# rubenwiersma/gravo_mg

Hardware: AMD Instinct MI355X
Metric: V-cycle wall time (ms per V-cycle incl. residual check) + solve-to-1e-4 iterations, 3M-vertex Poisson (lower is better)
Workload: dtype f64

## Files before the change

### gravo_mg_amd/cabi.py

```python
from __future__ import annotations

import ctypes as C
import os
from typing import List, Optional, Sequence, Tuple

import numpy as np
import scipy.sparse as sp

_HERE = os.path.dirname(os.path.abspath(__file__))
LIB_PATH = os.environ.get("GMG_LIB_PATH") or os.path.join(_HERE, "lib", "libgravomg_hip.so")

GMG_OK, GMG_ERR_INVALID, GMG_ERR_NO_DEVICE, GMG_ERR_HIP, GMG_ERR_STATE, GMG_ERR_NUMERIC, GMG_ERR_UNSUPPORTED = 0, -1, -2, -3, -4, -5, -6
DIVERGED = 1
SMOOTHER_MULTICOLOR_GS, SMOOTHER_JACOBI, SMOOTHER_CHEBYSHEV = 0, 1, 2
COARSE_HOST_LDLT, COARSE_DEVICE_INVERSE, COARSE_AUTO, COARSE_DEVICE_TRIANGLE = 0, 1, 2, 3

_STATUS_NAMES = {
    -1: "GMG_ERR_INVALID", -2: "GMG_ERR_NO_DEVICE", -3: "GMG_ERR_HIP", -4: "GMG_ERR_STATE",
    -5: "GMG_ERR_NUMERIC", -6: "GMG_ERR_UNSUPPORTED",
}


class GmgError(RuntimeError):
    def __init__(self, code: int, msg: str):
        super().__init__(f"{_STATUS_NAMES.get(code, code)}: {msg}")
        self.code = code


class GmgConfig(C.Structure):
    _fields_ = [
        ("device", C.c_int), ("smoother", C.c_int), ("jacobi_omega", C.c_double), ("pre_iters", C.c_int),
        ("post_iters", C.c_int), ("coarse_mode", C.c_int), ("use_graph", C.c_int), ("sigma", C.c_int),
        ("row_align", C.c_int), ("block_rows", C.c_int), ("block_lanes", C.c_int), ("block_from_level", C.c_int),
        ("device_setup", C.c_int), ("device_rap", C.c_int), ("reorder_fine", C.c_int), ("inner_precision", C.c_int), ("block_csr", C.c_int), ("host_threads", C.c_int),
        ("verbose", C.c_int), ("gs_omega", C.c_double), ("restrict_sigma", C.c_int), ("block_ep", C.c_int), ("dist_shard_levels", C.c_int), ("block_fine", C.c_int), ("fine_col16", C.c_int), ("stream_gate", C.c_int), ("dist_exchange", C.c_int), ("prepare_structure", C.c_int), ("fuse_restrict_sweep", C.c_int), ("speculate_head", C.c_int), ("uniform_slices", C.c_int), ("color_ahead", C.c_int),
        ("accelerate", C.c_int),
    ]


class GmgHierarchyOptions(C.Structure):
    _fields_ = [
        ("ratio", C.c_double), ("lower_bound", C.c_int), ("check_voronoi", C.c_int), ("nested", C.c_int),
        ("sampling", C.c_int), ("weighting", C.c_int), ("debug", C.c_int), ("full_clustering", C.c_int), ("use_device", C.c_int),
    ]


class GmgDeviceVectors(C.Structure):
    _fields_ = [
        ("rhs", C.c_void_p), ("rhs_row_stride", C.c_int64), ("rhs_col_stride", C.c_int64),
        ("x0", C.c_void_p), ("x0_row_stride", C.c_int64), ("x0_col_stride", C.c_int64),
        ("x", C.c_void_p), ("x_row_stride", C.c_int64), ("x_col_stride", C.c_int64),
    ]


_ip = C.POINTER(C.c_int)
_dp = C.POINTER(C.c_double)
_vp = C.c_void_p

SIGNATURES = {
    "gmg_config_default": (C.c_int, [C.POINTER(GmgConfig)]),
    "gmg_config_size": (C.c_int, []),
    "gmg_create": (C.c_int, [C.POINTER(GmgConfig), C.POINTER(_vp)]),
    "gmg_destroy": (None, [_vp]),
    "gmg_last_error": (C.c_char_p, [_vp]),
    "gmg_device_count": (C.c_int, []),
    "gmg_set_num_levels": (C.c_int, [_vp, C.c_int]),
    "gmg_set_prolongation": (C.c_int, [_vp, C.c_int, C.c_int, C.c_int, _ip, _ip, _dp]),
    "gmg_set_mass": (C.c_int, [_vp, C.c_int, _dp]),
    "gmg_set_system": (C.c_int, [_vp, C.c_int, _ip, _ip, _dp]),
    "gmg_num_levels": (C.c_int, [_vp]),
    "gmg_level_info": (C.c_int, [_vp, C.c_int, _ip, C.POINTER(C.c_int64), _ip, _ip]),
    "gmg_get_level_operator": (C.c_int, [_vp, C.c_int, _ip, _ip, _dp]),
    "gmg_get_level_ordering": (C.c_int, [_vp, C.c_int, _ip, _ip]),
    "gmg_get_level_blocks": (C.c_int, [_vp, C.c_int, _ip, _ip, C.POINTER(C.c_ubyte)]),
    "gmg_get_timing": (C.c_int, [_vp, C.c_char_p, _dp]),
    "gmg_smooth": (C.c_int, [_vp, C.c_int, _dp, _dp, C.c_int, C.c_int]),
    "gmg_residual": (C.c_int, [_vp, C.c_int, _dp, _dp, C.c_int, _dp]),
    "gmg_spmv": (C.c_int, [_vp, C.c_int, _dp, C.c_int, _dp]),
    "gmg_restrict": (C.c_int, [_vp, C.c_int, _dp, C.c_int, _dp]),
    "gmg_prolong_add": (C.c_int, [_vp, C.c_int, _dp, C.c_int, _dp]),
    "gmg_coarse_solve": (C.c_int, [_vp, _dp, C.c_int, _dp]),
    "gmg_residual_norm": (C.c_int, [_vp, _dp, _dp, C.c_int, C.c_int, _dp]),
    "gmg_vcycle": (C.c_int, [_vp, _dp, _dp, C.c_int]),
    "gmg_smooth_residual": (C.c_int, [_vp, C.c_int, _dp, _dp, C.c_int, C.c_int, C.c_int, _dp]),
    "gmg_solve": (C.c_int, [_vp, _dp, _dp, C.c_int, C.c_double, C.c_int, C.c_int, _ip, _dp, _dp]),
    "gmg_solve_x0_rhs": (C.c_int, [_vp, _dp, _dp, C.c_int, C.c_double, C.c_int, C.c_int, _ip, _dp, _dp]),
    "gmg_solve_device": (C.c_int, [_vp, C.POINTER(GmgDeviceVectors), C.c_int, C.c_double, C.c_int, C.c_int, _ip, _dp, _dp]),
    "gmg_set_system_values_device": (C.c_int, [_vp, C.c_void_p, C.c_int64]),
    "gmg_load_problem": (C.c_int, [_vp, _dp, _dp, C.c_int]),
    "gmg_run_cycles": (C.c_int, [_vp, C.c_int, C.c_int, _dp]),
    "gmg_fetch_solution": (C.c_int, [_vp, _dp]),
    "gmg_set_stream": (C.c_int, [_vp, _vp]),
    "gmg_dist_setup": (C.c_int, [_vp, C.c_int, C.c_int]),
    "gmg_dist_partition": (C.c_int, [_vp, C.c_int, C.c_int]),
    "gmg_dist_bind": (C.c_int, [_vp, _vp, _vp, _vp, C.c_int]),
    "gmg_dist_smooth_color": (C.c_int, [_vp, C.c_int]),
    "gmg_dist_residual_own": (C.c_int, [_vp]),
    "gmg_dist_coarse_cycle": (C.c_int, [_vp]),
    "gmg_dist_prolong_own": (C.c_int, [_vp]),
    "gmg_dist_norm_partial": (C.c_int, [_vp, C.c_int, _dp]),
    "gmg_dist_all_rows": (C.c_int, [_vp, C.c_int]),
    "gmg_dist_gather": (C.c_int, [_vp, C.c_void_p, C.c_void_p, C.c_int64, C.c_void_p]),
    "gmg_dist_scatter": (C.c_int, [_vp, C.c_void_p, C.c_void_p, C.c_void_p, C.c_int64, C.c_void_p]),
    "gmg_p2p_blob_bytes": (C.c_int, []),
    "gmg_p2p_prepare": (C.c_int, [_vp, C.c_int, C.c_int, C.c_int]),
    "gmg_p2p_export": (C.c_int, [_vp, C.c_void_p]),
    "gmg_p2p_connect": (C.c_int, [_vp, C.c_void_p]),
    "gmg_p2p_rccl_unique_id": (C.c_int, [C.c_void_p]),
    "gmg_p2p_connect_rccl": (C.c_int, [_vp, C.c_void_p]),
    "gmg_p2p_load": (C.c_int, [_vp, _dp, _dp]),
    "gmg_p2p_cycles": (C.c_int, [_vp, C.c_int, C.c_int, _dp]),
    "gmg_p2p_fetch": (C.c_int, [_vp, _dp]),
    "gmg_p2p_solve": (C.c_int, [_vp, _dp, _dp, C.c_double, C.c_int, C.c_int, C.POINTER(C.c_int), C.POINTER(C.c_double)]),
    "gmg_p2p_stat": (C.c_int, [_vp, C.c_char_p, _dp]),
    "gmg_p2p_set_smoother": (C.c_int, [_vp, C.c_int]),
    "gmg_p2p_set_fences": (C.c_int, [_vp, C.c_int]),
    "gmg_hierarchy_options_default": (C.c_int, [C.POINTER(GmgHierarchyOptions)]),
    "gmg_hierarchy_build": (C.c_int, [_dp, C.c_int, _ip, C.c_int, C.POINTER(GmgHierarchyOptions), C.POINTER(_vp)]),
    "gmg_hierarchy_destroy": (None, [_vp]),
# ... 118 lines not shown


def _pd(a: np.ndarray):
    return a.ctypes.data_as(_dp)


class Hierarchy:

    def __init__(self, pos, neigh, ratio=8.0, lower_bound=1000, check_voronoi=True, nested=False, sampling=0, weighting=0, debug=False, full_clustering=False, use_device=True):
        l = lib()
        pos = np.ascontiguousarray(pos, dtype=np.float64)
        neigh = np.ascontiguousarray(neigh, dtype=np.int32)
        if pos.ndim != 2 or pos.shape[1] != 3 or neigh.ndim != 2 or neigh.shape[0] != pos.shape[0]:
            raise ValueError("pos must be n x 3 and neigh n x K")
        opt = GmgHierarchyOptions()
        l.gmg_hierarchy_options_default(C.byref(opt))
        opt.ratio, opt.lower_bound, opt.check_voronoi, opt.nested = float(ratio), int(lower_bound), int(bool(check_voronoi)), int(bool(nested))
        opt.sampling, opt.weighting, opt.debug, opt.full_clustering = int(sampling), int(weighting), int(bool(debug)), int(bool(full_clustering))
        opt.use_device = int(use_device)
        self._h = _vp()
        rc = l.gmg_hierarchy_build(_pd(pos), pos.shape[0], _pi(neigh), neigh.shape[1], C.byref(opt), C.byref(self._h))
        if rc:
            raise GmgError(rc, "gmg_hierarchy_build failed (only Sampling.FASTDISK is supported)" if rc == GMG_ERR_UNSUPPORTED else "gmg_hierarchy_build failed")
        self.U: List[sp.csc_matrix] = []
        for k in range(l.gmg_hierarchy_num_levels(self._h)):
            nf, nc, nnz = C.c_int(), C.c_int(), C.c_int()
            l.gmg_hierarchy_level_shape(self._h, k, C.byref(nf), C.byref(nc), C.byref(nnz))
            colptr = np.empty(nc.value + 1, np.int32); rowidx = np.empty(nnz.value, np.int32); val = np.empty(nnz.value, np.float64)
            l.gmg_hierarchy_get_prolongation(self._h, k, _pi(colptr), _pi(rowidx), _pd(val))
            self.U.append(sp.csc_matrix((val, rowidx, colptr), shape=(nf.value, nc.value)))
        self.samples, self.nearest, self.points = [], [], []
        for k, u in enumerate(self.U):
            s_ = np.empty(u.shape[1], np.int32); n_ = np.empty(u.shape[0], np.int32); p_ = np.empty((u.shape[1], 3), np.float64)
            if l.gmg_hierarchy_get_samples(self._h, k, _pi(s_)) or l.gmg_hierarchy_get_nearest(self._h, k, _pi(n_)) or l.gmg_hierarchy_get_points(self._h, k, _pd(p_)):
                raise GmgError(GMG_ERR_INVALID, "hierarchy getters failed")
            self.samples.append(s_); self.nearest.append(n_); self.points.append(p_)
        self.triangles = []
        for k in range(len(self.U)):
            cnt = C.c_int()
            l.gmg_hierarchy_get_triangles(self._h, k, None, C.byref(cnt))
            t = np.empty((cnt.value, 3), np.int32)
            if cnt.value:
                l.gmg_hierarchy_get_triangles(self._h, k, _pi(t), C.byref(cnt))
            self.triangles.append(t)
        cnt = C.c_int()
        l.gmg_hierarchy_get_fine_order(self._h, None, C.byref(cnt))
        self.fine_order = None
        if cnt.value:
            self.fine_order = np.empty(cnt.value, np.int32)
            l.gmg_hierarchy_get_fine_order(self._h, _pi(self.fine_order), C.byref(cnt))

    def row_kinds(self, k: int) -> np.ndarray:
        out = np.zeros(4, np.int32)
        if lib().gmg_hierarchy_debug_row_kinds(self._h, int(k), _pi(out)):
            raise GmgError(GMG_ERR_INVALID, "gmg_hierarchy_debug_row_kinds failed")
        return out

    def timing(self, key: str) -> float:
        out = C.c_double()
        rc = lib().gmg_hierarchy_get_timing(self._h, key.encode(), C.byref(out))
        if rc:
            raise KeyError(key)
        return out.value

    TIMING_KEYS = ("n_vertices", "hierarchy", "sampling", "cluster", "next_neighborhood", "next_positions",
                   "triangle_finding", "triangle_selection", "PDS", "levels")

    def timings(self) -> dict:
        return {k: self.timing(k) for k in self.TIMING_KEYS}

    def __del__(self):
        try:
            if getattr(self, "_h", None):
                lib().gmg_hierarchy_destroy(self._h)
                self._h = None
        except Exception:
            pass


class Engine:

    def __init__(self, smoother=SMOOTHER_MULTICOLOR_GS, pre_iters=2, post_iters=2, jacobi_omega=0.67,
                 coarse_mode=COARSE_AUTO, use_graph=False, sigma=0, row_align=64, block_rows=64, block_from_level=1, block_lanes=0,
                 device_setup=True, device_rap=True, reorder_fine=2, inner_precision=0, block_csr=True, device=0, verbose=False, gs_omega=None, block_ep=None, restrict_sigma=None, dist_shard_levels=None, block_fine=None, fine_col16=None, stream_gate=None, prepare_structure=None, dist_exchange=None, fuse_restrict_sweep=None, speculate_head=None, uniform_slices=None, color_ahead=None, accelerate=0):
        l = lib()
        cfg = GmgConfig()
        l.gmg_config_default(C.byref(cfg))
        cfg.device, cfg.smoother, cfg.jacobi_omega = int(device), int(smoother), float(jacobi_omega)
        cfg.pre_iters, cfg.post_iters, cfg.coarse_mode = int(pre_iters), int(post_iters), int(coarse_mode)
        cfg.use_graph, cfg.sigma, cfg.row_align, cfg.verbose = int(bool(use_graph)), int(sigma), int(row_align), int(bool(verbose))
        cfg.block_rows, cfg.block_from_level, cfg.block_lanes = int(block_rows), int(block_from_level), int(block_lanes)
        cfg.device_setup, cfg.device_rap, cfg.reorder_fine = int(bool(device_setup)), int(bool(device_rap)), int(reorder_fine)
        cfg.inner_precision, cfg.block_csr = int(inner_precision), int(bool(block_csr))
        if gs_omega is not None:
            cfg.gs_omega = float(gs_omega)
        if block_ep is not None:
            cfg.block_ep = int(bool(block_ep))
        if restrict_sigma is not None:
            cfg.restrict_sigma = int(restrict_sigma)
        if dist_shard_levels is not None:
            cfg.dist_shard_levels = int(dist_shard_levels)
        if block_fine is not None:
            cfg.block_fine = int(bool(block_fine))
        if fine_col16 is not None:
            cfg.fine_col16 = int(bool(fine_col16))
        if stream_gate is not None:
            cfg.stream_gate = int(bool(stream_gate))
        if prepare_structure is not None:
            cfg.prepare_structure = int(bool(prepare_structure))
        if fuse_restrict_sweep is not None:
            cfg.fuse_restrict_sweep = int(bool(fuse_restrict_sweep))
        if speculate_head is not None:
            cfg.speculate_head = int(bool(speculate_head))
        if uniform_slices is not None:
            cfg.uniform_slices = int(bool(uniform_slices))
        if color_ahead is not None:
            cfg.color_ahead = int(bool(color_ahead))
        if dist_exchange is not None:
            cfg.dist_exchange = int(dist_exchange)
        cfg.accelerate = int(accelerate)
        self._h = _vp()
        rc = l.gmg_create(C.byref(cfg), C.byref(self._h))
        if rc:
            raise GmgError(rc, "gmg_create failed (invalid configuration)")
        self._n0 = None
        self._sizes: List[int] = []
        self.pre_iters, self.post_iters = int(pre_iters), int(post_iters)
        self.gs_omega = float(cfg.gs_omega)

    @classmethod
    def borrow(cls, handle: int) -> "Engine":
        self = cls.__new__(cls)
        self._h = _vp(int(handle))
        self._borrowed = True
        self._n0 = None
        self._sizes = []
        self.pre_iters = self.post_iters = None
        self.gs_omega = None
        return self

    def _chk(self, rc: int):
        if rc:
            raise GmgError(rc, lib().gmg_last_error(self._h).decode())

    def close(self):
        if getattr(self, "_h", None):
            if not getattr(self, "_borrowed", False):
                lib().gmg_destroy(self._h)
            self._h = None

    def __del__(self):
        try:
            self.close()
        except Exception:
            pass

    def set_prolongations(self, U: Sequence, finalize: bool = True, fine_order=None, fine_graph=None):
        l = lib()
        self._chk(l.gmg_set_num_levels(self._h, len(U)))
        self._sizes = []
        for k, u in enumerate(U):
            u = _csc(u)
            self._chk(l.gmg_set_prolongation(self._h, k, u.shape[0], u.shape[1], _pi(u.indptr), _pi(u.indices), _pd(u.data)))
            if k == 0:
                self._sizes.append(u.shape[0])
            self._sizes.append(u.shape[1])
        if fine_order is not None and len(U):
            fo = np.ascontiguousarray(fine_order, dtype=np.int32)
            self._chk(l.gmg_set_fine_order(self._h, fo.shape[0], _pi(fo)))
        if fine_graph is not None and len(U):
            fg = np.ascontiguousarray(fine_graph, dtype=np.int32)
            self._chk(l.gmg_set_fine_graph(self._h, fg.shape[0], fg.shape[1], _pi(fg)))
        if finalize and len(U):
            self._chk(l.gmg_finalize_hierarchy(self._h))

    def use_hierarchy(self, hier: Hierarchy):
        self._chk(lib().gmg_use_hierarchy(self._h, hier._h))
        self._sizes = [hier.U[0].shape[0]] + [u.shape[1] for u in hier.U] if hier.U else []

    def set_mass(self, mass_diag):
        m = np.ascontiguousarray(mass_diag, dtype=np.float64).ravel()
        self._chk(lib().gmg_set_mass(self._h, m.shape[0], _pd(m)))

    def set_system(self, lhs):
        a = _csc_layout(lhs)
        if a.shape[0] != a.shape[1]:
            raise ValueError("lhs must be square")
        self._chk(lib().gmg_set_system(self._h, a.shape[0], _pi(a.indptr), _pi(a.indices), _pd(a.data)))
        self._n0 = a.shape[0]

    @property
    def num_levels(self) -> int:
        return int(lib().gmg_num_levels(self._h))

    def level_info(self, k: int) -> dict:
        n, nnz, nc, npad = C.c_int(), C.c_int64(), C.c_int(), C.c_int()
        self._chk(lib().gmg_level_info(self._h, k, C.byref(n), C.byref(nnz), C.byref(nc), C.byref(npad)))
        return {"n": n.value, "nnz": nnz.value, "n_colors": nc.value, "n_pad": npad.value}

    def level_operator(self, k: int) -> sp.csc_matrix:
        info = self.level_info(k)
        colptr = np.empty(info["n"] + 1, np.int32); rowidx = np.empty(info["nnz"], np.int32); val = np.empty(info["nnz"], np.float64)
        self._chk(lib().gmg_get_level_operator(self._h, k, _pi(colptr), _pi(rowidx), _pd(val)))
# ... 429 lines not shown
```

### gravo_mg_amd/csrc/bindings.cpp

```cpp
#include <chrono>
#include <cstdio>
#include <cstdlib>
#include <pybind11/numpy.h>
#include <pybind11/pybind11.h>
#include <pybind11/stl.h>

#include <algorithm>
#include <atomic>
#include <cmath>
#include <cstdint>
#include <memory>
#include <stdexcept>
#include <string>
#include <thread>
#include <vector>

#include "multigrid_solver.h"

namespace py = pybind11;
using DenseIn = py::array_t<double, py::array::f_style | py::array::forcecast>;
using IntIn = py::array_t<int, py::array::c_style | py::array::forcecast>;

namespace {

// ... 202 lines not shown
        MGBS::MatrixXd x = b;
        solver->clearError();
        if (pardiso) throw std::runtime_error("direct_solve(pardiso=True): Pardiso (MKL) is not part of this build; use pardiso=False (sparse LDL^T)");
        solver->solve(A, b, x, 0);
        check();
        return from_dense(x);
    }

    py::list prolongation_matrices() {
        py::list out;
        for (const auto& u : solver->U) out.append(from_sparse(u));
        return out;
    }

    void set_prolongation_matrices(py::list U) {
        std::vector<MGBS::SparseMatrix> v;
        for (auto item : U) v.push_back(to_sparse(py::reinterpret_borrow<py::object>(item)));
        solver->U = v;
    }

    std::vector<std::vector<int>> sampling_indices() { return solver->samples; }
    std::vector<std::vector<size_t>> nearest_source() { return solver->nearestSource; }
    py::list level_points() {
        py::list out;
        for (const auto& P : solver->levelV) out.append(from_dense(P));
        return out;
    }
    py::list level_edges() { return py::list(); }
    std::vector<std::vector<int>> notrimap() { return solver->noTriFoundMap; }
    std::vector<std::vector<std::vector<int>>> all_triangles() { return solver->allTriangles; }
    py::list coarse_normals() { return py::list(); }

    void write_hierarchy_timing(std::string experiment, std::string file, bool write_headers) { MGBS::writeTiming(solver->hierarchyTiming, experiment, file, write_headers); }
    void write_solver_timing(std::string experiment, std::string file, bool write_headers) { MGBS::writeTiming(solver->solverTiming, experiment, file, write_headers); }
    void write_convergence(std::string file) { MGBS::writeConvergence(solver->convergence, file); }

    double residual(py::object lhs, DenseIn rhs, DenseIn solution, int type = 2) {
        MappedSparse mapped = map_system_matrix(lhs, symCache);
        MGBS::SparseMatrix& A = mapped.m;
        solver->clearError();
        double r = solver->residualCheck(A, to_dense(rhs), to_dense(solution), type);
        check();
        return r;
    }

    std::map<std::string, double> solver_timing() { return solver->solverTiming; }
    std::map<std::string, double> hierarchy_timing() { return solver->hierarchyTiming; }
    std::vector<std::tuple<double, double>> convergence() { return solver->convergence; }
    std::tuple<uintptr_t, long> prepare_system(py::object lhs) {
        MappedSparse mapped = map_system_matrix(lhs, symCache);
        gmg_handle h = nullptr;
        long gen = 0;
        solver->clearError();
        if (solver->prepareSystem(mapped.m, &h, &gen) != GMG_OK) { check(); throw std::runtime_error("prepare_system failed"); }
        return std::make_tuple((uintptr_t)h, gen);
    }
    uintptr_t engine_handle() { return (uintptr_t)solver->engineHandle(); }
    void invalidate_system() { solver->systemChangedExternally(); }
    void set_engine_option(const std::string& key, double value) {
        gmg_config& c = solver->engineConfig;
        if (key == "smoother") c.smoother = (int)value;
        else if (key == "jacobi_omega") c.jacobi_omega = value;
        else if (key == "gs_omega") c.gs_omega = value;
        else if (key == "coarse_mode") c.coarse_mode = (int)value;
        else if (key == "use_graph") c.use_graph = (int)value;
        else if (key == "block_rows") c.block_rows = (int)value;
        else if (key == "block_from_level") c.block_from_level = (int)value;
        else if (key == "device") c.device = (int)value;
        else if (key == "row_align") c.row_align = (int)value;
        else if (key == "block_lanes") c.block_lanes = (int)value;
        else if (key == "dist_shard_levels") c.dist_shard_levels = (int)value;
        else if (key == "block_fine") c.block_fine = (int)value;
        else if (key == "dist_rank") solver->distRank = (int)value;
        else if (key == "dist_world") solver->distWorld = (int)value;
        else if (key == "fine_col16") c.fine_col16 = (int)value;
        else if (key == "stream_gate") c.stream_gate = (int)value;
        else if (key == "fuse_restrict_sweep") c.fuse_restrict_sweep = (int)value;
        else if (key == "speculate_head") c.speculate_head = (int)value;
        else if (key == "uniform_slices") c.uniform_slices = (int)value;
        else if (key == "color_ahead") c.color_ahead = (int)value;
        else if (key == "dist_exchange") c.dist_exchange = (int)value;
        else if (key == "inner_precision") c.inner_precision = (int)value;
        else if (key == "accelerate") c.accelerate = (int)value;
        else throw std::invalid_argument("unknown engine option: " + key);
    }

#ifdef GMG_TESTING
    void test_report_diverged(int n) { solver->testReportDiverged = n; }
#endif

private:
    void check() {
        std::string now = solver->lastError();
        if (!now.empty()) throw std::runtime_error(now);
    }
    std::unique_ptr<MGBS::MultigridSolver> solver;
    SymmetryCache symCache;
};

PYBIND11_MODULE(gravomg_bindings, m) {
    m.doc() = "Multigrid solver bindings (MI355X-native V-cycle hot path)";

    py::enum_<Hierarchy>(m, "Hierarchy").value("OURS", OURS).value("SIG21", SIG21);
    py::enum_<Sampling>(m, "Sampling").value("FASTDISK", FASTDISK).value("POISSONDISK", POISSONDISK).value("FPS", FPS).value("RANDOM", RANDOM).value("MIS", MIS);
    py::enum_<Weighting>(m, "Weighting").value("BARYCENTRIC", BARYCENTRIC).value("UNIFORM", UNIFORM).value("INVDIST", INVDIST);

    py::class_<MultigridSolver>(m, "MultigridSolver")
        .def(py::init<DenseIn, IntIn, py::object, double, int, int, double, int, int, int, int, bool, bool, Sampling, Weighting, bool, DenseIn, bool, bool, bool, int, bool>())
        .def("construct_sig21_hierarchy", &MultigridSolver::construct_sig21_hierarchy, py::arg("F"))
        .def("toggle_hierarchy", &MultigridSolver::toggle_hierarchy, py::arg("hierarchy"))
        .def("solve", &MultigridSolver::solve, py::arg("lhs"), py::arg("rhs"))
        .def("direct_solve", &MultigridSolver::direct_solve, py::arg("lhs"), py::arg("rhs"), py::arg("pardiso"))
        .def("prolongation_matrices", &MultigridSolver::prolongation_matrices)
        .def("set_prolongation_matrices", &MultigridSolver::set_prolongation_matrices, py::arg("U"))
        .def("sampling_indices", &MultigridSolver::sampling_indices)
        .def("level_points", &MultigridSolver::level_points)
        .def("level_edges", &MultigridSolver::level_edges)
        .def("notrimap", &MultigridSolver::notrimap)
        .def("all_triangles", &MultigridSolver::all_triangles)
        .def("coarse_normals", &MultigridSolver::coarse_normals)
        .def("nearest_source", &MultigridSolver::nearest_source)
        .def("write_hierarchy_timing", &MultigridSolver::write_hierarchy_timing, py::arg("experiment"), py::arg("file"), py::arg("write_headers"))
        .def("write_solver_timing", &MultigridSolver::write_solver_timing, py::arg("experiment"), py::arg("file"), py::arg("write_headers"))
        .def("write_convergence", &MultigridSolver::write_convergence, py::arg("file"))
        .def("residual", &MultigridSolver::residual, py::arg("lhs"), py::arg("rhs"), py::arg("solution"), py::arg("type") = 2)
        .def("solver_timing", &MultigridSolver::solver_timing)
        .def("hierarchy_timing", &MultigridSolver::hierarchy_timing)
        .def("convergence", &MultigridSolver::convergence)
        .def("prepare_system", &MultigridSolver::prepare_system, py::arg("lhs"))
        .def("engine_handle", &MultigridSolver::engine_handle)
        .def("invalidate_system", &MultigridSolver::invalidate_system)
        .def("set_engine_option", &MultigridSolver::set_engine_option, py::arg("key"), py::arg("value"))
#ifdef GMG_TESTING
        .def("_test_report_diverged", &MultigridSolver::test_report_diverged, py::arg("n"))
#endif
        ;
}
```

### gravo_mg_amd/csrc/engine.hip

```cpp
#include <hip/hip_runtime.h>
#include <dlfcn.h>

#include <array>
#include <atomic>
#include <chrono>
#include <cmath>
#include <functional>
#include <future>
#include <cstdio>
#include <cstdlib>
#include <cstring>
#include <map>
#include <mutex>
#include <shared_mutex>
#include <string>
#include <vector>

#if !defined(__HIP_DEVICE_COMPILE__)
#include <execinfo.h>
#include <signal.h>
#include <unistd.h>
#endif

#include "../../include/gravomg_hip.h"
// ... 8 lines not shown
#include "setup_kernels.hip.hpp"
#include "hierarchy_kernels.hip.hpp"
#include "accel_kernels.hip.hpp"

using namespace gmg;
using clk = std::chrono::steady_clock;
static inline double ms_since(clk::time_point t0) { return std::chrono::duration<double, std::milli>(clk::now() - t0).count(); }

#if !defined(__HIP_DEVICE_COMPILE__)
namespace {
struct sigaction gmg_prev_action[32];
void gmg_fatal_signal(int sig) {
    void* frames[48];
    const int nf = backtrace(frames, 48);
    const char msg[] = "[gmg] fatal signal, native stack of the faulting thread:\n";
    (void)!write(2, msg, sizeof(msg) - 1);
    backtrace_symbols_fd(frames, nf, 2);
    if (sig > 0 && sig < 32) sigaction(sig, &gmg_prev_action[sig], nullptr); else signal(sig, SIG_DFL);
    raise(sig);
}
struct GmgSignalAid {
    GmgSignalAid() {
        if (!EnvSwitches::get().segv_backtrace) return;
        void* warm[4];
        (void)backtrace(warm, 4);
        struct sigaction sa;
        std::memset(&sa, 0, sizeof(sa));
        sa.sa_handler = gmg_fatal_signal;
        for (int sig : {SIGSEGV, SIGBUS, SIGABRT, SIGFPE}) sigaction(sig, &sa, &gmg_prev_action[sig]);
    }
} gmg_signal_aid;
}
#endif

#include "engine_state.hip.hpp"
#include "engine_setup.hip.hpp"
#include "engine_cycle.hip.hpp"
#include "engine_part.hip.hpp"
#include "engine_system.hip.hpp"

int gate_unwound(gmg_handle h);
#define GMG_CATCH_H                                                                                             \
    catch (const std::exception& e_) { if (h) (void)gate_unwound(h); return h ? fail(h, GMG_ERR_STATE, std::string("exception: ") + e_.what()) : GMG_ERR_STATE; } \
    catch (...) { if (h) (void)gate_unwound(h); return h ? fail(h, GMG_ERR_STATE, "unknown exception") : GMG_ERR_STATE; }
#define GMG_CATCH_0                                              \
    catch (...) { return GMG_ERR_STATE; }

void p2p_release_handle(gmg_handle h);


extern "C" {

int gmg_config_size(void) { return (int)sizeof(gmg_config); }

int gmg_config_default(gmg_config* cfg) try {
    if (!cfg) return GMG_ERR_INVALID;
    std::memset(cfg, 0, sizeof(*cfg));
    cfg->device = 0;
    cfg->smoother = GMG_SMOOTHER_MULTICOLOR_GS;
    cfg->jacobi_omega = 0.67;
    cfg->pre_iters = 2;
    cfg->post_iters = 2;
    cfg->coarse_mode = GMG_COARSE_AUTO;
    cfg->use_graph = 0;
    cfg->sigma = 0;
    cfg->row_align = 64;
    cfg->block_rows = 64;
    cfg->block_from_level = 1;
    cfg->block_lanes = 0;
    cfg->device_setup = 1;
    cfg->device_rap = 1;
    cfg->reorder_fine = 2;
    cfg->inner_precision = 0;
    cfg->block_csr = 1;
    cfg->host_threads = 0;
    cfg->verbose = 0;
    cfg->block_ep = 1;
    cfg->dist_shard_levels = 2;
    cfg->fine_col16 = 1;
    cfg->stream_gate = 1;
    cfg->prepare_structure = 1;
    cfg->fuse_restrict_sweep = 1;
    cfg->speculate_head = 1;
    cfg->uniform_slices = 1;
    cfg->color_ahead = 1;
    cfg->dist_exchange = 0;
    cfg->block_fine = 1;
    cfg->restrict_sigma = 64;
    cfg->gs_omega = 1.35;
    cfg->accelerate = 0;
    return GMG_OK;
} GMG_CATCH_0

int gmg_host_threads(void) try { return hw_threads(); } GMG_CATCH_0

int gmg_device_count(void) try {
    int n = 0;
    if (hipGetDeviceCount(&n) != hipSuccess) return 0;
    return n;
} GMG_CATCH_0

int gmg_create(const gmg_config* cfg, gmg_handle* out) try {
    if (!out) return GMG_ERR_INVALID;
    gmg_config c;
    if (cfg) c = *cfg; else gmg_config_default(&c);
    if (c.sigma < 0 || c.sigma % 64 || c.restrict_sigma < 0 || c.restrict_sigma % 64 || c.row_align <= 0 || c.row_align % 64 || c.pre_iters < 0 || c.post_iters < 0 ||
        c.reorder_fine < 0 || c.reorder_fine > 2 || c.inner_precision < 0 || c.inner_precision > 1 || c.block_rows < 0 || c.block_rows > gmgk::kBlockRows || c.block_rows % 64 || c.block_from_level < 0 || !(c.gs_omega > 0.0 && c.gs_omega < 2.0) || c.dist_shard_levels < 1 || c.dist_shard_levels > 2 || c.block_fine < 0 || c.block_fine > 1 || c.dist_exchange < 0 || c.dist_exchange > 2 ||
        (c.block_lanes != 0 && c.block_lanes != 1 && c.block_lanes != 4) || (c.block_lanes != 1 && c.block_rows > gmgk::kQuadBlockRows)) return GMG_ERR_INVALID;
    if (c.accelerate < 0 || c.accelerate > gmg::kAccelMaxDepth) return GMG_ERR_INVALID;
    if (c.smoother < GMG_SMOOTHER_MULTICOLOR_GS || c.smoother > GMG_SMOOTHER_CHEBYSHEV) return GMG_ERR_INVALID;
    if (c.accelerate > 0 && c.inner_precision) return GMG_ERR_UNSUPPORTED;
    gmg_handle h = new gmg_solver_s();
    h->cfg = c;
    if (h->cfg.host_threads <= 0) h->cfg.host_threads = hw_threads();
    int ndev = gmg_device_count();
    if (ndev > 0 && c.device >= 0 && c.device < ndev && hipSetDevice(c.device) == hipSuccess &&
        hipStreamCreateWithFlags(&h->stream, hipStreamNonBlocking) == hipSuccess) {
        h->has_device = true;
        h->own_stream = h->stream;
        { int cus = 0; if (hipDeviceGetAttribute(&cus, hipDeviceAttributeMultiprocessorCount, c.device) == hipSuccess && cus > 0) h->n_cus = cus; else (void)hipGetLastError(); }
        (void)hipEventCreate(&h->ev0);
        (void)hipEventCreate(&h->ev1);
        if (hipStreamCreateWithFlags(&h->aux_stream, hipStreamNonBlocking) != hipSuccess) { h->aux_stream = nullptr; (void)hipGetLastError(); }
        if (hipEventCreateWithFlags(&h->aux_ev, hipEventDisableTiming) != hipSuccess) { h->aux_ev = nullptr; (void)hipGetLastError(); }
        if (hipMalloc((void**)&h->d_aux_err, sizeof(int)) != hipSuccess) { h->d_aux_err = nullptr; (void)hipGetLastError(); }
        h->poll = EnvSwitches::get().poll;
        (void)ensure_bounce(h);
    }
    *out = h;
    return GMG_OK;
} GMG_CATCH_0

void gmg_destroy(gmg_handle h) {
    if (!h) return;
    PoolScope pool_scope_(&h->pool);
    if (h->has_device) {
        (void)hipSetDevice(h->cfg.device);
        (void)hipStreamSynchronize(h->stream);
        p2p_release_handle(h);
        drop_system(h);
        drop_device_transfers(h);
        h->d_stage = {}; h->d_partials = {}; h->d_norm = {}; h->d_watch = {};
        if (h->h_pinned) (void)sync_hipHostFree(h->h_pinned);
        for (int i = 0; i < 2; ++i) { if (h->h_stage[i]) (void)sync_hipHostFree(h->h_stage[i]); if (h->h_stage_ev[i]) (void)hipEventDestroy(h->h_stage_ev[i]); }
        for (hipEvent_t& e : h->h_chunk_ev) if (e) (void)hipEventDestroy(e);
        if (h->h_norm) (void)sync_hipHostFree(h->h_norm);
        if (h->h_flag) (void)sync_hipHostFree(h->h_flag);
        if (h->ev0) (void)hipEventDestroy(h->ev0);
        if (h->ev1) (void)hipEventDestroy(h->ev1);
        if (h->aux_ev) (void)hipEventDestroy(h->aux_ev);
        if (h->aux_stream) { (void)hipStreamSynchronize(h->aux_stream); (void)sync_hipStreamDestroy(h->aux_stream); }
        if (h->d_aux_err) (void)sync_hipFree(h->d_aux_err);
        drop_rap_order(h);
        for (int i = 0; i < 2; ++i) { if (h->bounce[i]) (void)sync_hipHostFree(h->bounce[i]); if (h->bounce_ev[i]) (void)hipEventDestroy(h->bounce_ev[i]); }
        for (hipEvent_t e : h->prof_ev) (void)hipEventDestroy(e);
        (void)sync_hipStreamDestroy(h->own_stream);
        h->pool.trim();
    }
    delete h;
}

const char* gmg_last_error(gmg_handle h) { return h ? h->err.c_str() : "null handle"; }

int gmg_set_num_levels(gmg_handle h, int L) try {
    if (!h || L < 0 || L > 64) return h ? fail(h, GMG_ERR_INVALID, "invalid level count") : GMG_ERR_INVALID;
    PoolScope pool_scope_(&h->pool);
// ... 300 lines not shown
    if (!e || !x || d <= 0) return fail(h, GMG_ERR_INVALID, "bad arguments");
    if ((rc = ensure_vectors(h, d))) return rc;
    Level& l = h->lv[k];
    if ((rc = to_device(h, k + 1, e, d, h->lv[k + 1].x))) return rc;
    if ((rc = to_device(h, k, x, d, l.x))) return rc;
    launch_prolong_add<double>(h, l, h->lv[k + 1], d, h->lv[k + 1].x, l.x);
    h->loaded_d = 0;
    return to_host(h, k, l.x, d, x);
} GMG_CATCH_H

int gmg_coarse_solve(gmg_handle h, const double* rc_in, int d, double* e) try {
    NEED_DEVICE();
    int rc = check_level(h, h->L, true);
    if (rc) return rc;
    if (!rc_in || !e || d <= 0) return fail(h, GMG_ERR_INVALID, "bad arguments");
    if ((rc = ensure_vectors(h, d))) return rc;
    Level& c = h->lv[h->L];
    if ((rc = to_device(h, h->L, rc_in, d, c.b))) return rc;
    if (h->coarse_device) enqueue_coarse_device<double>(h, d);
    else if ((rc = coarse_host_roundtrip<double>(h, d))) return rc;
    h->loaded_d = 0;
    return to_host(h, h->L, c.x, d, e);
} GMG_CATCH_H

int gmg_residual_norm(gmg_handle h, const double* b, const double* x, int d, int type, double* out) try {
    NEED_DEVICE();
    int rc = check_level(h, 0, false);
    if (rc) return rc;
    if ((rc = check_whole_system(h))) return rc;
    if (!b || !x || !out || d <= 0) return fail(h, GMG_ERR_INVALID, "bad arguments");
    if ((rc = check_norm_type(h, type))) return rc;
    if ((rc = ensure_vectors(h, d))) return rc;
    Level& l = h->lv[0];
    if ((rc = to_device(h, 0, b, d, l.b))) return rc;
    if ((rc = to_device(h, 0, x, d, l.x))) return rc;
    if ((rc = launch_norm(h, d, type))) return rc;
    if ((rc = wait_norm(h))) return rc;
    h->loaded_d = 0;
    *out = norm_from_sums(h->h_norm, d, type);
    return GMG_OK;
} GMG_CATCH_H


int gmg_load_problem(gmg_handle h, const double* b, const double* x0, int d) try {
    NEED_DEVICE();
    int rc = check_level(h, 0, false);
    if (rc) return rc;
    if (!b || !x0 || d <= 0) return fail(h, GMG_ERR_INVALID, "bad arguments");
    auto tl = clk::now();
    if ((rc = ensure_vectors(h, d))) return rc;
    h->timing["load_vectors"] = ms_since(tl); tl = clk::now();
    Level& l = h->lv[0];
    bool same = x0 == b;
    std::future<bool> compared;
    if (!same) {
        const size_t cnt = (size_t)l.n * d;
        const int threads = std::min(h->cfg.host_threads, 16);
        compared = std::async(std::launch::async, [b, x0, cnt, threads] {
            std::atomic<bool> differ{false};
            parallel_ranges((int)std::min<size_t>(cnt >> 12, 1 << 20) + 1, threads, [&](int lo, int hi, int) {
                const size_t a = (size_t)lo << 12, e = std::min(cnt, (size_t)hi << 12);
                if (a < e && !differ.load(std::memory_order_relaxed) && std::memcmp(b + a, x0 + a, sizeof(double) * (e - a)) != 0) differ = true;
            }, 2);
            return !differ.load();
        });
    }
    rc = to_device(h, 0, b, d, l.b);
    if (compared.valid()) same = compared.get();
    if (rc) return rc;
    h->timing["load_b"] = ms_since(tl); tl = clk::now();
    if (same) HIPCHK(hipMemcpyAsync(l.x, l.b, sizeof(double) * (size_t)l.n_pad * d, hipMemcpyDeviceToDevice, h->stream));
    else if ((rc = to_device(h, 0, x0, d, l.x))) return rc;
    h->timing["load_x"] = ms_since(tl); tl = clk::now();
    if (h->cfg.inner_precision && (rc = launch_residual_to_f32(h, d, -1))) return rc;
    HIPCHK(hipStreamSynchronize(h->stream));
    h->timing["load_sync"] = ms_since(tl);
    h->loaded_d = d;
    return GMG_OK;
} GMG_CATCH_H

namespace {
inline bool loop_enqueues_heads(gmg_handle h, int d, bool wanted) {
    if (!wanted || !head_eligible(h, d)) return false;
    h->timing["heads_enqueued"] += 0.0; h->timing["head_decision_differs"] += 0.0;
    return true;
}
}

int gmg_run_cycles(gmg_handle h, int n_cycles, int stop_type, double* residues) try {
    NEED_DEVICE();
    if (h->loaded_d <= 0) return fail(h, GMG_ERR_STATE, "no problem loaded (gmg_load_problem)");
    if (n_cycles < 0) return fail(h, GMG_ERR_INVALID, "bad cycle count");
    int rc;
    if ((rc = check_whole_system(h))) return rc;
    if (stop_type >= 0 && (rc = check_norm_type(h, stop_type))) return rc;
    const int d = h->loaded_d;
    HelperScope helper_scope(h, d);
    const bool heads = loop_enqueues_heads(h, d, stop_type >= 0);
    CycleWatch watch{0, 0.0, stop_type, 0};
    bool head_done = false;
    for (int i = 0; i < n_cycles; ++i) {
        watch.cycles_done = i + 1;
        if ((rc = vcycle_resident(h, d, stop_type, head_done, heads ? &watch : nullptr))) return rc;
        if (stop_type >= 0) {
            head_done = heads && i + 1 < n_cycles && enqueue_head(h, d);
            if ((rc = wait_norm(h))) return rc;
            if (residues) residues[i] = norm_from_sums(h->h_norm, d, stop_type);
        }
    }
    HIPCHK(hipStreamSynchronize(h->stream));
    return GMG_OK;
} GMG_CATCH_H

int gmg_profile_cycle(gmg_handle h, int stop_type, int reps, double* ms_out, int n_out) try {
    NEED_DEVICE();
    if (h->loaded_d <= 0) return fail(h, GMG_ERR_STATE, "no problem loaded (gmg_load_problem)");
    const int L = h->L;
    if (!ms_out || n_out < L + 2 || reps <= 0) return fail(h, GMG_ERR_INVALID, "bad arguments (ms_out needs levels + 2 entries)");
    if (h->cfg.use_graph) return fail(h, GMG_ERR_UNSUPPORTED, "leg profiling needs stream launches (use_graph = 0)");
    int rc;
    if ((rc = check_whole_system(h))) return rc;
    if ((rc = check_norm_type(h, stop_type))) return rc;
    const int d = h->loaded_d;
    HelperScope helper_scope(h, d);
    std::vector<double> acc((size_t)L + 2, 0.0);
    for (int i = 0; i < reps; ++i) {
        h->prof_on = true; h->prof_n = 0;
        rc = vcycle_resident(h, d, stop_type);
        h->prof_on = false;
        if (rc) return rc;
        if ((rc = wait_norm(h))) return rc;
        HIPCHK(hipStreamSynchronize(h->stream));
        if (h->prof_n != 2 * L + 3) return fail(h, GMG_ERR_STATE, "unexpected number of leg boundaries");
        auto span = [&](int a, int b) { float ms = 0.f; (void)hipEventElapsedTime(&ms, h->prof_ev[a], h->prof_ev[b]); return (double)ms; };
        for (int k = 0; k < L; ++k) acc[k] += span(k, k + 1) + span(L + 1 + (L - 1 - k), L + 2 + (L - 1 - k));
        acc[L] += span(L, L + 1);
        acc[L + 1] += span(2 * L + 1, 2 * L + 2);
    }
    for (int k = 0; k < L + 2; ++k) ms_out[k] = acc[k] / reps;
    return GMG_OK;
} GMG_CATCH_H

int gmg_fetch_solution(gmg_handle h, double* x) try {
    NEED_DEVICE();
    if (h->loaded_d <= 0) return fail(h, GMG_ERR_STATE, "no problem loaded (gmg_load_problem)");
    if (!x) return fail(h, GMG_ERR_INVALID, "bad arguments");
    return to_host(h, 0, h->lv[0].x, h->loaded_d, x);
} GMG_CATCH_H

int gmg_vcycle(gmg_handle h, const double* b, double* x, int d) try {
    int rc = gmg_load_problem(h, b, x, d);
    if (rc) return rc;
    if ((rc = gmg_run_cycles(h, 1, -1, nullptr))) return rc;
    return gmg_fetch_solution(h, x);
} GMG_CATCH_H

extern "C++" {
template <class Load, class Fetch>
static int solve_common(gmg_handle h, const char* bad_args, int d, double tol, int stop_type, int max_iter, int* iters_out, double* residue_out, double* conv,
                        Load&& load, Fetch&& fetch) {
    NEED_DEVICE();
    int rc;
    if (bad_args) return fail(h, GMG_ERR_INVALID, bad_args);
    if ((rc = check_whole_system(h))) return rc;
    if ((rc = check_norm_type(h, stop_type))) return rc;
    auto t_all = clk::now();
    HelperScope helper_scope(h, d);
    if ((rc = load())) return rc;
    h->timing["solve_load"] = ms_since(t_all);
    h->timing["coarse_host_ms"] = 0.0;
    auto t0 = clk::now();
    const int accel = h->cfg.accelerate;
    int confirmations = 0;
    Level& l0 = h->lv[0];
    auto accel_step = [&](SolveRule& rule, double& residue, int&) -> int {
        if ((rc = vcycle_resident(h, d, -1))) return rc;
        launch_spmv<double>(h, l0, d, 1, l0.b, l0.x, l0.r);
        if ((rc = launch_accel_step(h, d, stop_type, rule.cycles))) return rc;
        if ((rc = wait_norm(h))) return rc;
        residue = norm_from_sums(h->h_norm, d, stop_type);
        if (rule_goes_on(rule_after(rule, residue))) return GMG_OK;
        const double recurrence = residue;
        if ((rc = launch_norm(h, d, stop_type))) return rc;
        if ((rc = wait_norm(h))) return rc;
        residue = norm_from_sums(h->h_norm, d, stop_type);
        ++confirmations;
        rule = rule_confirmed(rule, recurrence, residue, rule_floor(h->h_norm, d, stop_type));
        if (rule_goes_on(rule_after(rule, residue))) launch_spmv<double>(h, l0, d, 1, l0.b, l0.x, h->accel.r);
        return GMG_OK;
    };
    const bool heads = loop_enqueues_heads(h, d, accel == 0);
    CycleWatch watch{1, tol, stop_type, 0};
    bool head_done = false;
    auto plain_step = [&](const SolveRule& rule, double& residue, int& device_go) -> int {
        watch.cycles_done = rule.cycles + 1;
        const bool head = heads && rule.cycles + 2 <= rule.max_iter;
        if ((rc = vcycle_resident(h, d, stop_type, head_done, heads ? &watch : nullptr))) return rc;
        head_done = head && enqueue_head(h, d);
        if ((rc = wait_norm(h))) return rc;
        residue = norm_from_sums(h->h_norm, d, stop_type);
        if (head) device_go = __atomic_load_n(h->h_flag + 1, __ATOMIC_ACQUIRE) != 0;
        if (device_go == 0) head_done = false;
        return GMG_OK;
    };
    int verdict;
    if (accel > 0) {
        if ((rc = ensure_accel(h))) return rc;
        HIPCHK(hipMemsetAsync(h->accel.scal, 0, sizeof(double) * ((size_t)9 * h->accel.d + 1), h->stream));
        HIPCHK(hipMemcpyAsync(h->accel.xk, l0.x, sizeof(double) * (size_t)l0.n_pad * d, hipMemcpyDeviceToDevice, h->stream));
        launch_spmv<double>(h, l0, d, 1, l0.b, l0.x, h->accel.r);
        verdict = solve_loop(h, tol, max_iter, t0, conv, h->cfg.verbose, iters_out, residue_out, accel_step);
    } else
        verdict = solve_loop(h, tol, max_iter, t0, conv, h->cfg.verbose, iters_out, residue_out, plain_step);
    if (verdict < 0) return verdict;
    h->timing["accelerate"] = accel;
    h->timing["accel_confirmations"] = confirmations;
    double guard_steps = 0.0;
    if (accel > 0) {
        HIPCHK(hipMemcpyAsync(&guard_steps, h->accel.scal + (size_t)8 * h->accel.d, sizeof(double), hipMemcpyDeviceToHost, h->stream));
        HIPCHK(hipStreamSynchronize(h->stream));
    }
    h->timing["accel_guard_steps"] = guard_steps;
    auto t_f = clk::now();
    if ((rc = fetch())) return rc;
    h->timing["solve_fetch"] = ms_since(t_f);
    h->timing["solve_call"] = ms_since(t_all);
    h->timing["solver_total"] = h->timing["setup_total"] + h->timing["solve_call"];
    return verdict;
}
}

static int solve_host(gmg_handle h, const double* rhs, const double* x0, double* x, int d, double tol, int stop_type, int max_iter, int* iters_out,
                      double* residue_out, double* conv) {
    return solve_common(h, rhs && x0 && x ? nullptr : "bad arguments", d, tol, stop_type, max_iter, iters_out, residue_out, conv,
                        [&] { return gmg_load_problem(h, rhs, x0, d); }, [&] { return gmg_fetch_solution(h, x); });
}

int gmg_solve(gmg_handle h, const double* rhs, double* x, int d, double tol, int stop_type, int max_iter, int* iters_out,
              double* residue_out, double* conv) try {
    return solve_host(h, rhs, x, x, d, tol, stop_type, max_iter, iters_out, residue_out, conv);
} GMG_CATCH_H

int gmg_solve_x0_rhs(gmg_handle h, const double* rhs, double* x, int d, double tol, int stop_type, int max_iter, int* iters_out,
                     double* residue_out, double* conv) try {
    return solve_host(h, rhs, rhs, x, d, tol, stop_type, max_iter, iters_out, residue_out, conv);
} GMG_CATCH_H

static int load_problem_device(gmg_handle h, const gmg_device_vectors& v, int d) {
    int rc = check_level(h, 0, false);
    if (rc) return rc;
    Level& l = h->lv[0];
    if (const char* why = device_vectors_fault(&v, l.n, d)) return fail(h, GMG_ERR_INVALID, why);
    if ((rc = check_device_vectors(h, v, l.n, d))) return rc;
    if ((rc = ensure_vectors(h, d))) return rc;
    launch_permute_in2_strided(h, l, v, d);
    if (h->cfg.inner_precision && (rc = launch_residual_to_f32(h, d, -1))) return rc;
    h->loaded_d = d;
    return GMG_OK;
}

int gmg_solve_device(gmg_handle h, const gmg_device_vectors* v, int d, double tol, int stop_type, int max_iter, int* iters_out,
                     double* residue_out, double* conv) try {
    return solve_common(h, device_vectors_fault(v, 1, d), d, tol, stop_type, max_iter, iters_out, residue_out, conv,
                        [&] { return load_problem_device(h, *v, d); },
                        [&] {
                            launch_permute_out_strided(h, h->lv[0], *v, d);
                            HIPCHK(hipStreamSynchronize(h->stream));
                            return (int)GMG_OK;
                        });
} GMG_CATCH_H

int gmg_set_system_values_device(gmg_handle h, const double* d_val, int64_t nnz) try {
    NEED_DEVICE();
    int rc;
    if (h->live != LiveSystem::system) return fail(h, GMG_ERR_STATE, h->live == LiveSystem::placeholder ? "no system set: the handle holds the prepared structure only (call gmg_set_system first)" : "no system set (call gmg_set_system first)");
    if ((rc = check_whole_system(h))) return rc;
    if (!h->live_key_valid || !h->refill_ready || (int)h->lv.size() != h->L + 1 || !refresh_possible(h) || h->live_from_copy)
        return fail(h, GMG_ERR_STATE, "the live system cannot be refreshed in place (set up by the host planner, or from arrays that were not in canonical storage): use gmg_set_system");
    Level& l0 = h->lv[0];
    if (nnz != l0.nnz) return fail(h, GMG_ERR_STATE, "nnz = " + std::to_string(nnz) + " but the live system stores " + std::to_string(l0.nnz) + " entries");
    if (!d_val) return fail(h, GMG_ERR_INVALID, "d_val is NULL");
    if ((rc = check_device_block(h, d_val, nnz - 1, "d_val"))) return rc;
    auto t_all = clk::now();
    HIPCHK(hipSetDevice(h->cfg.device));
    if (l0.ord.blocked && h->cfg.block_from_level >= 1) {
// ... 796 lines not shown
```

### gravo_mg_amd/csrc/engine_cycle.hip.hpp

```cpp
#pragma once

namespace {


#define DISPATCH_D(dc, ...)              \
    switch (dc) {                        \
        case 1: { constexpr int D = 1; __VA_ARGS__; } break; \
        case 2: { constexpr int D = 2; __VA_ARGS__; } break; \
        case 3: { constexpr int D = 3; __VA_ARGS__; } break; \
        default: { constexpr int D = 4; __VA_ARGS__; } break; \
    }

#define DISPATCH_C16(mode, ...)          \
    switch (mode) {                      \
        case 1: { constexpr int C16 = 1; __VA_ARGS__; } break; \
        case 2: { constexpr int C16 = 2; __VA_ARGS__; } break; \
        case 3: { constexpr int C16 = 3; __VA_ARGS__; } break; \
        case 4: { constexpr int C16 = 4; __VA_ARGS__; } break; \
        default: { constexpr int C16 = 0; __VA_ARGS__; } break; \
    }

#define DISPATCH_FLAG(NAME, cond, ...)   \
    { if (cond) { constexpr bool NAME = true; __VA_ARGS__; } else { constexpr bool NAME = false; __VA_ARGS__; } }

#define DISPATCH_ONE_OF(NAME, v, A, B, C, ...)   \
    { if ((v) == (A)) { constexpr int NAME = A; __VA_ARGS__; } else if ((v) == (B)) { constexpr int NAME = B; __VA_ARGS__; } else { constexpr int NAME = C; __VA_ARGS__; } }

template <class F>
inline void for_col_chunks(int d, F&& f) {
    for (int c0 = 0; c0 < d; c0 += 4) f(c0, std::min(4, d - c0));
}

template <class T> struct Prec;
template <> struct Prec<double> {
    static const double* val(const DevSell& s) { return s.val; }
    static const double* diag(const Level& l) { return l.diag; }
    static const double* bcval(const Level& l) { return l.bc_val; }
    static const double* epval(const Level& l) { return l.ep_val; }
    static const double* eeval(const Level& l) { return l.ee_val; }
    static double* x(Level& l) { return l.x; }
    static double* b(Level& l) { return l.b; }
    static double* r(Level& l) { return l.r; }
    static double* tmp(Level& l) { return l.tmp; }
};
template <> struct Prec<float> {
    static const float* val(const DevSell& s) { return s.val32; }
    static const float* diag(const Level& l) { return l.diag32; }
    static const float* bcval(const Level& l) { return l.bc_val32; }
    static const float* epval(const Level& l) { return l.ep_val32; }
    static const float* eeval(const Level& l) { return l.ee_val32; }
    static float* x(Level& l) { return l.x32; }
    static float* b(Level& l) { return l.b32; }
    static float* r(Level& l) { return l.r32; }
    static float* tmp(Level& l) { return l.tmp32; }
};

template <class T>
struct SmoothAsk {
    bool from_zero = false;
    bool first_done = false;
    bool head_done = false;
    T* res_out = nullptr;
    bool res_il = false;
    int norm_type = -1;
    T* il_out = nullptr;
};
template <class T>
struct SmoothDone {
    int res_from = 0;
    int norm_blocks = 0;
    const T* prev = nullptr;
    bool prev_valid = false;
    bool il_written = false;
};

template <class T>
int fold_norm(gmg_handle, Level&, int, bool, int, int, int) { return 0; }
template <>
int fold_norm<double>(gmg_handle h, Level& l, int d, bool last_launch, int sb, int se, int type) {
    if (!last_launch || type < 0 || &l != &h->lv[0] || d > 4 || l.ord.n_colors < 2 || se != l.Aoff.n_slices) return 0;
    const double* w = type == 1 ? h->d_minv : (type == 2 ? h->d_mass : nullptr);
    const int nblk = grid_for(se - sb), first = norm_grid(sb);
    if ((size_t)(first + nblk) > (size_t)h->partial_blocks) return 0;
    DISPATCH_D(d, DISPATCH_C16(l.Aoff.c16_sel(), hipLaunchKernelGGL((gmgk::gs_color_norm<D, C16>), dim3(nblk), dim3(gmgk::kBlock), 0, h->stream, l.Aoff.slice_ptr,
                                     l.Aoff.col, l.Aoff.val, l.diag, l.b, l.x, l.n_pad, sb, se, h->cfg.gs_omega, w, h->d_partials + (size_t)first * 2 * d,
                                     l.Aoff.col16, l.Aoff.win_base, l.Aoff.c16_arg())));
    return nblk;
}

template <class T>
int fold_residual(gmg_handle, Level&, int, bool, int, int, T*, bool) { return 0; }
template <>
int fold_residual<double>(gmg_handle h, Level& l, int d, bool last_launch, int sb, int se, double* out, bool il) {
    if (!last_launch || !out || &l != &h->lv[0] || d > 4 || l.ord.n_colors < 2 || se != l.Aoff.n_slices || sb <= 0) return 0;
    DISPATCH_D(d, DISPATCH_C16(l.Aoff.c16_sel(), DISPATCH_FLAG(YI, il, hipLaunchKernelGGL((gmgk::gs_color_residual<D, C16, (YI && D > 1)>), dim3(grid_for(se - sb)),
                                     dim3(gmgk::kBlock), 0, h->stream, l.Aoff.slice_ptr, l.Aoff.col, l.Aoff.val, l.diag, l.b, l.x, out, l.n_pad, sb, se,
                                     h->cfg.gs_omega, l.Aoff.col16, l.Aoff.win_base, l.Aoff.c16_arg()))));
    return sb;
}

inline bool polled(gmg_handle h);

template <class T>
T level_omega(gmg_handle h, const Level& l) { return &l == &h->lv[0] ? (T)h->cfg.gs_omega : (T)1.0; }

template <class T>
void launch_gs_color(gmg_handle h, Level& l, int c0, int dc, int sb, int se, T omega, const unsigned long long* plain_rows = nullptr, const int* go = nullptr) {
    const int ld = l.n_pad;
    T* x = Prec<T>::x(l);
    const T* b = Prec<T>::b(l);
    if (&l == &h->lv[0]) {
        DISPATCH_D(dc, DISPATCH_C16(l.Aoff.c16_sel(), DISPATCH_FLAG(OM, plain_rows != nullptr, hipLaunchKernelGGL((gmgk::gs_color<T, D, C16 + 1, (OM && sizeof(T) == 8)>),
                                          dim3(grid_for(se - sb)), dim3(gmgk::kBlock), 0, h->stream, l.Aoff.slice_ptr, l.Aoff.col, Prec<T>::val(l.Aoff), Prec<T>::diag(l),
                                          b + (size_t)c0 * ld, x + (size_t)c0 * ld, ld, sb, se, 1, omega, l.Aoff.col16, l.Aoff.win_base, l.Aoff.c16_arg(), plain_rows, go))));
    } else {
        DISPATCH_D(dc, hipLaunchKernelGGL((gmgk::gs_color<T, D, 0>), dim3(grid_for(se - sb)), dim3(gmgk::kBlock), 0, h->stream,
                                          l.Aoff.slice_ptr, l.Aoff.col, Prec<T>::val(l.Aoff), Prec<T>::diag(l), b + (size_t)c0 * ld,
                                          x + (size_t)c0 * ld, ld, sb, se, 1, omega));
    }
}

inline int first_color(const Level& l) {
    for (int c = 0; c < l.ord.n_colors; ++c)
        if (l.ord.color_begin[c + 1] / 64 > l.ord.color_begin[c] / 64) return c;
    return -1;
}

inline bool head_eligible(gmg_handle h, int d) {
    return h->cfg.speculate_head && polled(h) && !h->cfg.inner_precision && h->cfg.smoother == GMG_SMOOTHER_MULTICOLOR_GS && h->cfg.pre_iters > 0 && h->L >= 1 &&
           !h->lv[0].ord.blocked && h->lv[0].ord.n_colors >= 2 && first_color(h->lv[0]) >= 0 && first_color(h->lv[0]) < h->lv[0].ord.n_colors - 1 && d >= 1 && d <= 4 &&
           !h->partitioned && h->part_world <= 1 && h->d_watch && !h->prof_on;
}
inline bool enqueue_head(gmg_handle h, int d) {
    Level& l = h->lv[0];
    const int c = first_color(l);
    launch_gs_color<double>(h, l, 0, d, l.ord.color_begin[c] / 64, l.ord.color_begin[c + 1] / 64, level_omega<double>(h, l), nullptr, reinterpret_cast<const int*>(h->d_watch + 1));
    h->timing["heads_enqueued"] += 1.0;
    return true;
}

template <class T>
SmoothDone<T> launch_gs_sweeps(gmg_handle h, Level& l, int d, int iters, const SmoothAsk<T>& ask) {
    SmoothDone<T> done;
    const int c_head = ask.head_done ? first_color(l) : -1;
    for (int it = 0; it < iters; ++it)
        for_col_chunks(d, [&](int c0, int dc) {
            for (int c = 0; c < l.ord.n_colors; ++c) {
                int sb = l.ord.color_begin[c] / 64, se = l.ord.color_begin[c + 1] / 64;
                if (se <= sb) continue;
                if (it == 0 && c0 == 0 && c == c_head) continue;
                const bool last_launch = it == iters - 1 && c == l.ord.n_colors - 1;
                if (const int nblk = fold_norm<T>(h, l, d, last_launch, sb, se, ask.norm_type)) { done.norm_blocks = nblk; continue; }
                if (const int from = fold_residual<T>(h, l, d, last_launch, sb, se, ask.res_out, ask.res_il)) { done.res_from = from; continue; }
                launch_gs_color<T>(h, l, c0, dc, sb, se, level_omega<T>(h, l));
            }
        });
    return done;
}

template <class T>
void launch_jacobi_sweeps(gmg_handle h, Level& l, int d, int iters) {
    const int ld = l.n_pad;
    T* in = Prec<T>::x(l); T* out = Prec<T>::tmp(l);
    const T* b = Prec<T>::b(l);
    for (int it = 0; it < iters; ++it) {
        for_col_chunks(d, [&](int c0, int dc) {
            DISPATCH_D(dc, hipLaunchKernelGGL((gmgk::jacobi_sweep<T, D>), dim3(grid_for(l.Aoff.n_slices)), dim3(gmgk::kBlock), 0, h->stream,
                                              l.Aoff.slice_ptr, l.Aoff.col, Prec<T>::val(l.Aoff), Prec<T>::diag(l), b + (size_t)c0 * ld,
                                              (in ? in + (size_t)c0 * ld : nullptr), out + (size_t)c0 * ld, ld, l.Aoff.n_slices, (T)h->cfg.jacobi_omega, 1));
        });
        std::swap(in, out);
    }
    if (in != Prec<T>::x(l)) (void)hipMemcpyAsync(Prec<T>::x(l), in, sizeof(T) * (size_t)ld * d, hipMemcpyDeviceToDevice, h->stream);
}

template <class T>
void launch_cheby_steps(gmg_handle h, Level& l, int d, int iters) {
    const int ld = l.n_pad;
    T* in = Prec<T>::x(l); T* out = Prec<T>::tmp(l);
    const T* b = Prec<T>::b(l);
    T* p = Prec<T>::r(l);
    const int c16 = &l == &h->lv[0] ? l.Aoff.c16_sel() : 0;
    const double ratio = cheby_ratio(h);
    for (int it = 0; it < iters; ++it) {
        const ChebyStep st = cheby_step_coeffs(l.cheby_lambda, ratio, it);
        for_col_chunks(d, [&](int c0, int dc) {
            DISPATCH_D(dc, DISPATCH_C16(c16, DISPATCH_FLAG(FIRST, it == 0, hipLaunchKernelGGL((gmgk::cheby_step<T, D, FIRST, C16>), dim3(grid_for(l.Aoff.n_slices)),
                                              dim3(gmgk::kBlock), 0, h->stream, l.Aoff.slice_ptr, l.Aoff.col, Prec<T>::val(l.Aoff), Prec<T>::diag(l), b + (size_t)c0 * ld,
                                              in + (size_t)c0 * ld, out + (size_t)c0 * ld, p + (size_t)c0 * ld, ld, l.Aoff.n_slices, (T)st.c1, (T)st.c2, 1, l.Aoff.col16,
                                              l.Aoff.win_base, l.Aoff.c16_arg()))));
        });
        std::swap(in, out);
    }
    if (in != Prec<T>::x(l)) (void)hipMemcpyAsync(Prec<T>::x(l), in, sizeof(T) * (size_t)ld * d, hipMemcpyDeviceToDevice, h->stream);
}

constexpr int64_t kEpResidentBytes = (int64_t)128 << 20;
inline bool ep_streams(const Level& l) { return l.ee_nnz * 12 + l.ep_nnz * 10 > kEpResidentBytes; }

template <class T>
void launch_block_sweep_range(gmg_handle h, Level& l, int d, const T* in, T* out, int b0, int nb, const int* begin_table = nullptr,
                              const int* ncolors_table = nullptr, T* out_il = nullptr) {
    const int ld = l.n_pad;
    const T* b = Prec<T>::b(l);
    const int* blk_begin = begin_table ? begin_table : l.d_blk_begin + b0;
    const int* blk_ncolors = ncolors_table ? ncolors_table : l.d_blk_ncolors + b0;
    if (nb <= 0) return;
    for_col_chunks(d, [&](int c0, int dc) {
        if (l.use_ep) {
            const int vgrid = (nb + 7) / 8 * 8;
            DISPATCH_D(dc, DISPATCH_FLAG(STREAM, ep_streams(l), hipLaunchKernelGGL((gmgk::gs_block_ep<T, D, STREAM>), dim3(vgrid), dim3(64),
                                              gmgk::ep_lds_bytes<T>(D, l.ep_cap_e, l.ep_cap_l), h->stream, begin_table, blk_ncolors, l.d_row_color, l.ep_ptr, l.ep_col,
                                              Prec<T>::epval(l), l.ee_ptr, l.ee_col, Prec<T>::eeval(l), Prec<T>::diag(l), b + (size_t)c0 * ld,
                                              (in ? in + (size_t)c0 * ld : nullptr), out + (size_t)c0 * ld, ld, l.ep_cap_e, l.ep_cap_l, nb, b0, vgrid, out_il)));
        } else if (l.use_bcsr && d > 1) {
            DISPATCH_D(dc, hipLaunchKernelGGL((gmgk::gs_block_csrout<T, D, (D == 1 ? 32 : 24)>), dim3(nb), dim3(64),
                                              (size_t)l.bc_cap * (sizeof(T) + sizeof(int)) + (size_t)D * 64 * sizeof(T), h->stream, blk_begin,
                                              blk_ncolors, l.d_row_color, l.Ain.slice_ptr, l.ain_col16, Prec<T>::val(l.Ain), l.bc_ptr, l.bc_col,
                                              Prec<T>::bcval(l), Prec<T>::diag(l), b + (size_t)c0 * ld, (in ? in + (size_t)c0 * ld : nullptr), out + (size_t)c0 * ld,
                                              ld, l.bc_cap));
        } else if (l.Ain.lpr == 4) {
            DISPATCH_D(dc, hipLaunchKernelGGL((gmgk::gs_block4<T, D, 8>), dim3(nb), dim3(4 * h->cfg.block_rows), 0, h->stream, blk_begin,
                                              blk_ncolors, l.d_row_color, l.Ain.slice_ptr, l.ain_col16, Prec<T>::val(l.Ain), l.Aout.slice_ptr,
                                              l.Aout.col, Prec<T>::val(l.Aout), Prec<T>::diag(l), b + (size_t)c0 * ld, (in ? in + (size_t)c0 * ld : nullptr),
                                              out + (size_t)c0 * ld, ld));
        } else {
            DISPATCH_D(dc, hipLaunchKernelGGL((gmgk::gs_block<T, D, (D == 1 ? 32 : 24)>), dim3(nb), dim3(h->cfg.block_rows), 0, h->stream, blk_begin,
                                              blk_ncolors, l.d_row_color, l.Ain.slice_ptr, l.ain_col16, Prec<T>::val(l.Ain), l.Aout.slice_ptr,
                                              l.Aout.col, Prec<T>::val(l.Aout), Prec<T>::diag(l), b + (size_t)c0 * ld, (in ? in + (size_t)c0 * ld : nullptr),
                                              out + (size_t)c0 * ld, ld));
        }
    });
}
// ... 103 lines not shown
}
template <class T>
void launch_restrict(gmg_handle h, Level& fine, Level& coarse, int d, const T* src, T* dst, bool src_il = false) {
    if (fine.R.lpr == 4) launch_restrict_lpr<T, 4>(h, fine, coarse, d, src, dst, src_il);
    else launch_restrict_lpr<T, 1>(h, fine, coarse, d, src, dst, src_il);
}

template <class T>
int restrict_sweep0_kind(gmg_handle h, const Level& fine, const Level& coarse, int d, bool src_il) {
    if (!h->cfg.fuse_restrict_sweep || pointwise_smoother(h->cfg) || h->cfg.pre_iters <= 0 || d > 4) return 0;
    if (!coarse.ord.blocked || fine.R.lpr != 4 || !(h->cfg.restrict_sigma == 0 || h->cfg.restrict_sigma == 64)) return 0;
    if (coarse.use_ep) return (coarse.n_pad == 64 * coarse.ord.n_blocks() && fine.R.n_slices == 4 * coarse.ord.n_blocks()) ? 1 : 0;
    if (!(coarse.use_bcsr && d > 1) && coarse.Ain.lpr == 4 && fine.R.c16_mode == 0 && !src_il && fine.R.n_slices * 16 == coarse.n_pad) return 2;
    return 0;
}
template <class T>
void launch_restrict_sweep0(gmg_handle h, Level& fine, Level& coarse, int d, const T* src, bool src_il, int kind, const int* blk_list = nullptr, int nb_list = 0) {
    const int nb = blk_list ? nb_list : coarse.ord.n_blocks();
    if (kind == 2) {
        DISPATCH_D(d, hipLaunchKernelGGL((gmgk::gs_block4<T, D, 8, true>), dim3(nb), dim3(4 * h->cfg.block_rows), 0, h->stream, coarse.d_blk_begin, coarse.d_blk_ncolors,
                                         coarse.d_row_color, coarse.Ain.slice_ptr, coarse.ain_col16, Prec<T>::val(coarse.Ain), coarse.Aout.slice_ptr, coarse.Aout.col,
                                         Prec<T>::val(coarse.Aout), Prec<T>::diag(coarse), (const T*)nullptr, (const T*)nullptr, Prec<T>::tmp(coarse), coarse.n_pad,
                                         fine.R.slice_ptr, fine.R.col, Prec<T>::val(fine.R), fine.R.row_of, src, fine.n_pad, Prec<T>::b(coarse)));
        return;
    }
    const int vgrid = (nb + 7) / 8 * 8;
    const size_t lds_sweep = gmgk::ep_lds_bytes<T>(d, 0, coarse.ep_cap_l);
    const size_t lds = lds_sweep + (size_t)d * 64 * sizeof(T);
    DISPATCH_D(d, DISPATCH_C16(fine.R.c16_sel(), DISPATCH_FLAG(STREAM, ep_streams(coarse), DISPATCH_FLAG(XI, src_il,
                  hipLaunchKernelGGL((gmgk::restrict_sweep0<T, D, STREAM, C16, (XI && D > 1)>), dim3(vgrid), dim3(256), lds, h->stream, fine.R.slice_ptr, fine.R.col,
                                     Prec<T>::val(fine.R), fine.R.row_of, src, fine.n_pad, fine.R.col16, fine.R.win_base, fine.R.c16_arg(), Prec<T>::b(coarse),
                                     coarse.d_blk_ncolors, coarse.d_row_color, coarse.ep_ptr, coarse.ep_col, Prec<T>::epval(coarse), Prec<T>::diag(coarse),
                                     Prec<T>::tmp(coarse), coarse.n_pad, nb, vgrid, (int)lds_sweep, blk_list)))));
}

template <class T>
void launch_prolong_add(gmg_handle h, Level& fine, Level& coarse, int d, const T* src, T* dst, bool src_il = false, int sb = 0, int se = -1, int c16 = -1) {
    const bool il = src_il && d > 1 && d <= 4;
    if (se < 0) se = fine.P.n_slices;
    if (c16 < 0) c16 = fine.P.c16_sel();
    for_col_chunks(d, [&](int c0, int dc) {
        DISPATCH_D(dc, DISPATCH_C16(c16, DISPATCH_FLAG(XI, il, hipLaunchKernelGGL((gmgk::transfer<T, D, 1, 1, C16, (XI && D > 1)>), dim3(grid_for(se - sb)), dim3(gmgk::kBlock), 0,
                                          h->stream, fine.P.slice_ptr, fine.P.col, Prec<T>::val(fine.P), (const int*)nullptr, src + (size_t)c0 * coarse.n_pad, coarse.n_pad,
                                          dst + (size_t)c0 * fine.n_pad, fine.n_pad, sb, se, 1, fine.P.col16, fine.P.win_base, fine.P.c16_arg()))));
    });
}
template <class T>
void launch_prolong_add_list(gmg_handle h, Level& fine, Level& coarse, int d, const T* src, T* dst, const int* slices, int n_list) {
    for_col_chunks(d, [&](int c0, int dc) {
        DISPATCH_D(dc, hipLaunchKernelGGL((gmgk::transfer_list<T, D, 1, 1>), dim3(grid_for(n_list)), dim3(gmgk::kBlock), 0, h->stream, fine.P.slice_ptr, fine.P.col,
                                          Prec<T>::val(fine.P), (const int*)nullptr, src + (size_t)c0 * coarse.n_pad, coarse.n_pad, dst + (size_t)c0 * fine.n_pad,
                                          fine.n_pad, slices, n_list));
    });
}

constexpr unsigned kPolledHostFlags = hipHostMallocCoherent | hipHostMallocMapped;
inline bool polled(gmg_handle h) { return !h->cfg.use_graph && h->poll && h->h_flag; }

int wait_flag(gmg_handle h, int slot) {
    const unsigned long long want = h->flag_seq[slot];
    auto t0 = clk::now();
    double next_query_ms = 20.0;
    for (unsigned spin = 1;; ++spin) {
        if (__atomic_load_n(h->h_flag + 8 * slot, __ATOMIC_ACQUIRE) == want) return GMG_OK;
        if ((spin & 4095u) == 0 && ms_since(t0) > next_query_ms) {
            hipError_t q = hipStreamQuery(h->stream);
            if (q == hipSuccess) {
                if (__atomic_load_n(h->h_flag + 8 * slot, __ATOMIC_ACQUIRE) != want) { h->poll = false; h->timing["poll_disabled"] = 1.0; }
                return GMG_OK;
            }
            if (q != hipErrorNotReady) HIPCHK(q);
            next_query_ms += 20.0;
        }
        __builtin_ia32_pause();
    }
}

int wait_norm(gmg_handle h) {
    if (polled(h)) return wait_flag(h, 0);
    HIPCHK(hipStreamSynchronize(h->stream));
    return GMG_OK;
}

struct CycleWatch { int mode; double tol; int type; int cycles_done; };

void launch_reduce(gmg_handle h, int nblk, int dc, int c0, bool last, const double* partials = nullptr, const CycleWatch* decide = nullptr) {
    if (!partials) partials = h->d_partials;
    if (polled(h)) {
        gmgk::SolveWatch watch{nullptr, nullptr, nullptr, 0.0, 0, 0, 0, 0};
        if (decide && last && c0 == 0 && h->d_watch)
            watch = gmgk::SolveWatch{reinterpret_cast<int*>(h->d_watch + 1), h->h_flag + 1, h->d_watch, decide->tol, decide->mode, decide->type, dc, decide->cycles_done};
        hipLaunchKernelGGL(gmgk::reduce_partials, dim3(1), dim3(gmgk::kReduceBlock), 0, h->stream, partials, nblk, 2 * dc, h->h_norm + 2 * c0,
                           last ? h->h_flag : nullptr, last ? ++h->flag_seq[0] : 0ull, (int)EnvSwitches::get().publish_fenced, watch);
    }
    else
        hipLaunchKernelGGL(gmgk::reduce_partials, dim3(1), dim3(gmgk::kReduceBlock), 0, h->stream, partials, nblk, 2 * dc, h->d_norm + 2 * c0,
                           (unsigned long long*)nullptr, 0ull, 0);
}

int launch_norm(gmg_handle h, int d, int type, int folded = 0, const CycleWatch* decide = nullptr) {
    Level& l = h->lv[0];
    const double* w = type == 1 ? h->d_minv : (type == 2 ? h->d_mass : nullptr);
    const int n_slices = folded ? l.ord.color_begin[l.ord.n_colors - 1] / 64 : l.Aoff.n_slices;
    const int nblk = norm_grid(n_slices);
    const bool poll = polled(h);
    for_col_chunks(d, [&](int c0, int dc) {
        DISPATCH_D(dc, DISPATCH_C16(l.Aoff.c16_sel(), hipLaunchKernelGGL((gmgk::residual_norm_slices<D, 0, C16>), dim3(nblk), dim3(gmgk::kNormWaves * 64), 0, h->stream,
                                          l.Aoff.slice_ptr, l.Aoff.col, l.Aoff.val, l.diag, l.b + (size_t)c0 * l.n_pad, l.x + (size_t)c0 * l.n_pad, w,
                                          l.n_pad, n_slices, (float*)nullptr, h->d_partials, l.Aoff.col16, l.Aoff.win_base, l.Aoff.c16_arg())));
        launch_reduce(h, nblk + folded, dc, c0, c0 + 4 >= d, nullptr, decide);
    });
    if (!poll) HIPCHK(hipMemcpyAsync(h->h_norm, h->d_norm, sizeof(double) * 2 * d, hipMemcpyDeviceToHost, h->stream));
    return GMG_OK;
}

int ensure_vectors(gmg_handle h, int d) {
    if (d <= h->dcap) return GMG_OK;
    drop_graphs(h);
    unbind_level0(h);
    h->accel = {};
    auto vec = [&](auto& v, const Level& l, bool wanted) -> int {
        v.reset();
        if (!wanted) return GMG_OK;
        const size_t count = (size_t)l.n_pad * d;
        int rc = dev_alloc(h, v, count);
        if (rc == GMG_OK) HIPCHK(hipMemsetAsync(v, 0, sizeof(*v.get()) * count, h->stream));
        return rc;
    };
    for (auto& l : h->lv) {
        const bool tmp = pointwise_smoother(h->cfg) || l.ord.blocked, f32 = h->cfg.inner_precision != 0;
        int rc;
        if ((rc = vec(l.x, l, true)) || (rc = vec(l.b, l, true)) || (rc = vec(l.r, l, true)) || (rc = vec(l.tmp, l, tmp)) ||
            (rc = vec(l.x32, l, f32)) || (rc = vec(l.b32, l, f32)) || (rc = vec(l.r32, l, f32)) || (rc = vec(l.tmp32, l, f32 && tmp))) return rc;
    }
    Level& c = h->lv[h->L];
    size_t need = (size_t)c.n_pad * d * 2;
    if (need > h->pinned_cap) {
        if (h->h_pinned) (void)sync_hipHostFree(h->h_pinned);
        HIPCHK(hipHostMalloc((void**)&h->h_pinned, sizeof(double) * need, kPolledHostFlags));
        h->pinned_cap = need;
    }
    if (h->h_norm) (void)sync_hipHostFree(h->h_norm);
    HIPCHK(hipHostMalloc((void**)&h->h_norm, sizeof(double) * 2 * d, kPolledHostFlags));
    if (!h->h_flag) {
        HIPCHK(hipHostMalloc((void**)&h->h_flag, 256, kPolledHostFlags));
        std::memset(h->h_flag, 0, 256);
    }

    int rc;
    if ((rc = dev_alloc(h, h->d_norm, (size_t)2 * d))) return rc;
    if (!h->d_watch) {
        if ((rc = dev_alloc(h, h->d_watch, 2))) return rc;
        HIPCHK(hipMemsetAsync(h->d_watch, 0, 16, h->stream));
    }
    h->dcap = d;
    h->loaded_d = 0;
    return GMG_OK;
}

int ensure_stage(gmg_handle h, size_t n_doubles) {
    if (n_doubles <= h->stage_cap) return GMG_OK;
    int rc;
    if ((rc = dev_alloc(h, h->d_stage, n_doubles))) return rc;
    h->stage_cap = n_doubles;
    return GMG_OK;
}

int ensure_host_stage(gmg_handle h, size_t n_doubles) {
    if (n_doubles <= h->h_stage_cap) return GMG_OK;
    for (int i = 0; i < 2; ++i) {
        if (h->h_stage[i]) (void)sync_hipHostFree(h->h_stage[i]);
        h->h_stage[i] = nullptr;
        HIPCHK(hipHostMalloc((void**)&h->h_stage[i], sizeof(double) * n_doubles, hipHostMallocDefault));
        if (!h->h_stage_ev[i]) HIPCHK(hipEventCreateWithFlags(&h->h_stage_ev[i], hipEventDisableTiming));
    }
    h->h_stage_cap = n_doubles;
    return GMG_OK;
}

inline void threaded_copy(double* dst, const double* src, size_t n, int threads) {
    const int T = (int)std::min<size_t>(std::max(1, std::min(threads, 16)), n / 65536 + 1);
    if (T <= 1) { std::memcpy(dst, src, sizeof(double) * n); return; }
    parallel_ranges(T, T, [&](int t0, int t1, int) {
        for (int t = t0; t < t1; ++t) {
            size_t lo = n * t / T, hi = n * (t + 1) / T;
            std::memcpy(dst + lo, src + lo, sizeof(double) * (hi - lo));
        }
    }, 1);
}

constexpr int kXferChunks = 6;
inline size_t xfer_chunk(size_t cnt) { return std::max<size_t>((cnt + kXferChunks - 1) / kXferChunks, (size_t)1 << 17); }

int to_device(gmg_handle h, int k, const double* src, int d, double* dst) {
    Level& l = h->lv[k];
    const size_t n = (size_t)l.n, cnt = n * d;
    int rc = ensure_stage(h, cnt);
    if (rc) return rc;
    if ((rc = ensure_host_stage(h, n))) return rc;
    const size_t ch = xfer_chunk(n);
    for (int c = 0; c < d; ++c) {
        const int f = h->h_stage_flip;
        h->h_stage_flip ^= 1;
        HIPCHK(hipEventSynchronize(h->h_stage_ev[f]));
        for (size_t off = 0; off < n; off += ch) {
            const size_t len = std::min(ch, n - off);
            threaded_copy(h->h_stage[f] + off, src + c * n + off, len, h->cfg.host_threads);
            HIPCHK(hipMemcpyAsync(h->d_stage + c * n + off, h->h_stage[f] + off, sizeof(double) * len, hipMemcpyHostToDevice, h->stream));
        }
        HIPCHK(hipEventRecord(h->h_stage_ev[f], h->stream));
    }
    hipLaunchKernelGGL(gmgk::permute_in, dim3((l.n_pad + 255) / 256), dim3(256), 0, h->stream, h->d_stage, l.n, l.d_new2old, dst, l.n_pad, l.n_pad, d);
    return GMG_OK;
}

int to_host(gmg_handle h, int k, const double* src, int d, double* dst) {
// ... 21 lines not shown
        return GMG_OK;
    };
    if ((rc = issue(0))) return rc;
    for (int c = 0; c < d; ++c) {
        if (c + 1 < d && (rc = issue(c + 1))) return rc;
        const int f = c & 1;
        int nch = 0;
        for (size_t off = 0; off < n; off += ch, ++nch) {
            const size_t len = std::min(ch, n - off);
            HIPCHK(hipEventSynchronize(h->h_chunk_ev[f * kEvPerBuf + nch]));
            threaded_copy(dst + c * n + off, h->h_stage[f] + off, len, h->cfg.host_threads);
        }
    }
    HIPCHK(hipStreamSynchronize(h->stream));
    return GMG_OK;
}


#define DISPATCH_D_ANY(dc, ...)          \
    switch (dc) {                        \
        case 1: { constexpr int D = 1; __VA_ARGS__; } break; \
        case 2: { constexpr int D = 2; __VA_ARGS__; } break; \
        case 3: { constexpr int D = 3; __VA_ARGS__; } break; \
        case 4: { constexpr int D = 4; __VA_ARGS__; } break; \
        default: { constexpr int D = 0; __VA_ARGS__; } break; \
    }

int check_device_block(gmg_handle h, const void* p, int64_t extent, const char* what) {
    hipPointerAttribute_t attr;
    std::memset(&attr, 0, sizeof(attr));
    if (hipPointerGetAttributes(&attr, p) != hipSuccess) { (void)hipGetLastError(); return fail(h, GMG_ERR_INVALID, std::string(what) + " is not device memory (unknown to the HIP runtime: a host pointer?)"); }
    if (attr.type != hipMemoryTypeDevice || attr.isManaged) return fail(h, GMG_ERR_INVALID, std::string(what) + " is not plain device memory (host, pinned or managed memory)");
    if (attr.device != h->cfg.device) return fail(h, GMG_ERR_INVALID, std::string(what) + " lives on device " + std::to_string(attr.device) + ", the handle on device " + std::to_string(h->cfg.device));
    hipDeviceptr_t base = nullptr;
    size_t size = 0;
    if (hipMemGetAddressRange(&base, &size, (hipDeviceptr_t)p) != hipSuccess) { (void)hipGetLastError(); return GMG_OK; }
    const size_t off = (size_t)((const char*)p - (const char*)base);
    if (off > size || (size_t)(extent + 1) > (size - off) / sizeof(double)) return fail(h, GMG_ERR_INVALID, std::string(what) + " with these strides does not fit the allocation it points into");
    return GMG_OK;
}

int check_device_vectors(gmg_handle h, const gmg_device_vectors& v, int n, int d) {
    int rc;
    int64_t e = 0;
    (void)strided_extent(n, d, v.rhs_row_stride, v.rhs_col_stride, &e);
    if ((rc = check_device_block(h, v.rhs, e, "rhs"))) return rc;
    if (v.x0) {
        (void)strided_extent(n, d, v.x0_row_stride, v.x0_col_stride, &e);
        if ((rc = check_device_block(h, v.x0, e, "x0"))) return rc;
    }
    (void)strided_extent(n, d, v.x_row_stride, v.x_col_stride, &e);
    return check_device_block(h, v.x, e, "x");
}

void launch_permute_in2_strided(gmg_handle h, Level& l, const gmg_device_vectors& v, int d) {
    const dim3 grid((l.n_pad + 255) / 256);
    DISPATCH_D_ANY(d, DISPATCH_FLAG(X0, v.x0 != nullptr, hipLaunchKernelGGL((gmgk::permute_in2_strided<D, X0>), grid, dim3(256), 0, h->stream, v.rhs, v.rhs_row_stride,
                                        v.rhs_col_stride, v.x0, v.x0_row_stride, v.x0_col_stride, l.d_new2old, l.b, l.x, l.n_pad, l.n_pad, d)));
}

void launch_permute_out_strided(gmg_handle h, Level& l, const gmg_device_vectors& v, int d) {
    DISPATCH_D_ANY(d, hipLaunchKernelGGL((gmgk::permute_out_strided<D>), dim3((l.n_pad + 255) / 256), dim3(256), 0, h->stream, (const double*)l.x, l.n_pad, l.n_pad,
                                         l.d_new2old, v.x, v.x_row_stride, v.x_col_stride, d));
}


inline void prof_mark(gmg_handle h) {
    if (!h->prof_on) return;
    if ((size_t)h->prof_n >= h->prof_ev.size()) { hipEvent_t e = nullptr; if (hipEventCreate(&e) != hipSuccess) return; h->prof_ev.push_back(e); }
    (void)hipEventRecord(h->prof_ev[h->prof_n++], h->stream);
}

template <class T>
bool restrict_into(gmg_handle h, int k, int d, bool il) {
    Level& l = h->lv[k];
    Level& c = h->lv[k + 1];
    const int fused = (k + 1 < h->L && smooth_from_zero_ok(h, c, h->cfg.pre_iters)) ? restrict_sweep0_kind<T>(h, l, c, d, il) : 0;
    if (fused) { ++h->fused_restrictions; launch_restrict_sweep0<T>(h, l, c, d, Prec<T>::r(l), il, fused); }
    else launch_restrict<T>(h, l, c, d, Prec<T>::r(l), Prec<T>::b(c), il);
    return fused != 0;
}

template <class T = double>
void enqueue_down(gmg_handle h, int d, int k0 = 0, bool first_done = false, bool head_done = false) {
    const int L = h->L;
    for (int k = k0; k < L; ++k) {
        Level& l = h->lv[k];
        prof_mark(h);
        SmoothAsk<T> ask;
        ask.from_zero = k > 0 && smooth_from_zero_ok(h, l, h->cfg.pre_iters);
        if (k > 0 && !ask.from_zero) (void)hipMemsetAsync(Prec<T>::x(l), 0, sizeof(T) * (size_t)l.n_pad * d, h->stream);
        ask.first_done = first_done; ask.head_done = k == 0 && head_done;
        const bool il = k == 0 && d > 1 && d <= 4 && l.Aoff.lpr == 1;
        if (k == 0 && sizeof(T) == 8) { ask.res_out = Prec<T>::r(l); ask.res_il = il; }
        const SmoothDone<T> swept = launch_smooth<T>(h, l, d, h->cfg.pre_iters, ask);
        const int res_slices = (k == 0 && swept.res_from > 0) ? swept.res_from : -1;
        if (!(k > 0 && launch_residual_delta<T>(h, l, d, Prec<T>::r(l), swept)))
            launch_spmv<T>(h, l, d, 1, Prec<T>::b(l), Prec<T>::x(l), Prec<T>::r(l), res_slices, il);
        first_done = restrict_into<T>(h, k, d, il);
    }
    prof_mark(h);
}

template <class T = double>
int enqueue_up(gmg_handle h, int d, int k0 = 0, int norm_type = -1) {
    prof_mark(h);
    int norm_blocks = 0;
    bool il = false;
    for (int k = h->L - 1; k >= k0; --k) {
        Level& l = h->lv[k];
        const T* src = il ? Prec<T>::r(h->lv[k + 1]) : Prec<T>::x(h->lv[k + 1]);
        launch_prolong_add<T>(h, l, h->lv[k + 1], d, src, Prec<T>::x(l), il);
        SmoothAsk<T> ask;
        if (k == 1 && k0 == 0 && d > 1 && d <= 4 && h->cfg.post_iters > 0 && l.ord.blocked && l.use_ep && !pointwise_smoother(h->cfg))
            ask.il_out = Prec<T>::r(l);
        if (k == 0) ask.norm_type = norm_type;
        const SmoothDone<T> swept = launch_smooth<T>(h, l, d, h->cfg.post_iters, ask);
        il = swept.il_written; norm_blocks = swept.norm_blocks;
        prof_mark(h);
    }
    return norm_blocks;
}

inline void launch_cvt(gmg_handle h, const double* src, float* dst, size_t n) {
    if (n == 0) return;
    hipLaunchKernelGGL(gmgk::cvt_f64_to_f32, dim3((unsigned)((n + 255) / 256)), dim3(256), 0, h->stream, src, dst, (int64_t)n);
}
inline void launch_cvt(gmg_handle h, const float* src, double* dst, size_t n) {
    if (n == 0) return;
    hipLaunchKernelGGL(gmgk::cvt_f32_to_f64, dim3((unsigned)((n + 255) / 256)), dim3(256), 0, h->stream, src, dst, (int64_t)n);
}

#ifndef GMG_SYMV_ROWS
#define GMG_SYMV_ROWS 0
#endif
inline int symv_rows(int n, int d) {
    const int forced = EnvSwitches::get().symv_rows;
    if (forced == 1 || forced == 2 || forced == 4) return forced;
    if (GMG_SYMV_ROWS > 0) return GMG_SYMV_ROWS;
    (void)d;
    return n >= 3000 ? 2 : 1;
}
inline int symv_strides(int n, int d, int rows) {
    const int forced = EnvSwitches::get().symv_strides;
    if (forced == 2 || forced == 4 || forced == 8) return forced;
    (void)n; (void)d; (void)rows;
    return 4;
}

template <class T = double>
void enqueue_coarse_device(gmg_handle h, int d) {
    Level& c = h->lv[h->L];
    const size_t cnt = (size_t)c.n_pad * d;
    if (sizeof(T) == 4) launch_cvt(h, c.b32, c.b, cnt);
    if (h->coarse_triangle) {
        const int nb = tri_blocks(c.n);
        const bool nt = EnvSwitches::get().tri_nt;
        if (nb > 0) for_col_chunks(d, [&](int c0, int dc) {
            const double* b = c.b + (size_t)c0 * c.n_pad;
            double* x = c.x + (size_t)c0 * c.n_pad;
            DISPATCH_D(dc, DISPATCH_FLAG(NT, nt, hipLaunchKernelGGL((gmgk::tri_symv_items<D, NT>), dim3((unsigned)tri_item_count(nb)), dim3(gmgk::kBlock), 0, h->stream,
                                          (const double*)h->d_tri, (const int*)h->d_tri_perm, c.n, b, c.n_pad, h->d_tri_row, h->d_tri_col)));
            DISPATCH_D(dc, hipLaunchKernelGGL((gmgk::tri_symv_reduce<D>), dim3(nb), dim3(gmgk::kBlock), 0, h->stream, (const double*)h->d_tri_row,
                                          (const double*)h->d_tri_col, (const int*)h->d_tri_perm, c.n, nb, x, c.n_pad));
        });
        if (sizeof(T) == 4) launch_cvt(h, c.x, c.x32, cnt);
        return;
    }
    for_col_chunks(d, [&](int c0, int dc) {
        const int rows_per_wave = symv_rows(c.n, dc);
        const int per_block = gmgk::kWavesPerBlock * rows_per_wave;
        const dim3 grid((c.n + per_block - 1) / per_block);
        const int strides = symv_strides(c.n, dc, rows_per_wave);
        const double* b = c.b + (size_t)c0 * c.n_pad;
        double* x = c.x + (size_t)c0 * c.n_pad;
// ... 62 lines not shown

template <class T = double>
int coarse_host_begin(gmg_handle h, int d) {
    Level& c = h->lv[h->L];
    const size_t cnt = (size_t)c.n_pad * d;
    double* rc = h->h_pinned;
    double* e = h->h_pinned + cnt;
    if (sizeof(T) == 4) launch_cvt(h, c.b32, c.b, cnt);
    if (polled(h)) {
        hipLaunchKernelGGL(gmgk::publish_to_host, dim3(1), dim3(gmgk::kBlock), 0, h->stream, c.b, rc, (int)cnt, h->h_flag + 8, ++h->flag_seq[1], (int)EnvSwitches::get().publish_fenced);
        const bool gate_off = h->cfg.stream_gate == 0;
        if (h->gate_ok && h->gate_proven && !gate_off) {
            if (!h->gate_shared) { gate_mutex().lock_shared(); h->gate_shared = true; ++tl_gates_held; }
            if (hipStreamWaitValue64(h->stream, h->h_flag + 16, ++h->flag_seq[2], hipStreamWaitValueGte, ~0ull) == hipSuccess) {
                hipLaunchKernelGGL(gmgk::fetch_from_host, dim3((unsigned)std::min<size_t>(8, (cnt + gmgk::kBlock - 1) / gmgk::kBlock)), dim3(gmgk::kBlock), 0, h->stream,
                                   (const double*)e, c.x, (int)cnt);
                if (sizeof(T) == 4) launch_cvt(h, c.x, c.x32, cnt);
                h->coarse_pending = true; h->coarse_pending_d = d;
                return GMG_OK;
            }
            (void)hipGetLastError();
            if (h->gate_shared) { h->gate_shared = false; --tl_gates_held; gate_mutex().unlock_shared(); }
            h->gate_ok = false; --h->flag_seq[2]; h->timing["gate_disabled"] = 1.0;
        }
        int w = wait_flag(h, 1);
        if (w) return w;
        if (h->poll) h->gate_proven = true;
        if (!polled(h)) HIPCHK(hipStreamSynchronize(h->stream));
    } else {
        HIPCHK(hipMemcpyAsync(rc, c.b, sizeof(double) * cnt, hipMemcpyDeviceToHost, h->stream));
        HIPCHK(hipStreamSynchronize(h->stream));
    }
    coarse_host_solve(h, d);
    HIPCHK(hipMemcpyAsync(c.x, e, sizeof(double) * cnt, hipMemcpyHostToDevice, h->stream));
    if (sizeof(T) == 4) launch_cvt(h, c.x, c.x32, cnt);
    return GMG_OK;
}

template <class T = double>
int coarse_host_roundtrip(gmg_handle h, int d) {
    int rc = coarse_host_begin<T>(h, d);
    return rc ? rc : coarse_host_serve(h);
}

int launch_residual_to_f32(gmg_handle h, int d, int type) {
    Level& l = h->lv[0];
    const double* w = type == 1 ? h->d_minv : (type == 2 ? h->d_mass : nullptr);
    const int nblk = norm_grid(l.Aoff.n_slices);
    for_col_chunks(d, [&](int c0, int dc) {
        DISPATCH_D(dc, DISPATCH_C16(l.Aoff.c16_sel(), hipLaunchKernelGGL((gmgk::residual_norm_slices<D, 1, C16>), dim3(nblk), dim3(gmgk::kNormWaves * 64), 0, h->stream,
                                          l.Aoff.slice_ptr, l.Aoff.col, l.Aoff.val, l.diag, l.b + (size_t)c0 * l.n_pad, l.x + (size_t)c0 * l.n_pad, w, l.n_pad,
                                          l.Aoff.n_slices, l.b32 + (size_t)c0 * l.n_pad, h->d_partials, l.Aoff.col16, l.Aoff.win_base, l.Aoff.c16_arg())));
        launch_reduce(h, nblk, dc, c0, c0 + 4 >= d);
    });
    if (!polled(h)) HIPCHK(hipMemcpyAsync(h->h_norm, h->d_norm, sizeof(double) * 2 * d, hipMemcpyDeviceToHost, h->stream));
    return GMG_OK;
}

enum { G_DOWN = 1, G_UP = 2, G_FULL = 3 };

template <class F>
int run_graph(gmg_handle h, int key, F&& enqueue) {
    if (!h->cfg.use_graph) { enqueue(); return GMG_OK; }
    auto it = h->graphs.find(key);
    if (it == h->graphs.end()) {
        hipGraph_t g = nullptr;
        hipGraphExec_t ge = nullptr;
        auto tc = clk::now();
        HIPCHK(hipStreamBeginCapture(h->stream, hipStreamCaptureModeThreadLocal));
        enqueue();
        HIPCHK(hipStreamEndCapture(h->stream, &g));
        h->timing["graph_capture_ms"] += ms_since(tc);
        tc = clk::now();
        HIPCHK(hipGraphInstantiate(&ge, g, nullptr, nullptr, 0));
        h->timing["graph_instantiate_ms"] += ms_since(tc);
        (void)hipGraphDestroy(g);
        it = h->graphs.emplace(key, ge).first;
    }
    HIPCHK(hipGraphLaunch(it->second, h->stream));
    return GMG_OK;
}

template <class T>
int vcycle_legs(gmg_handle h, int d, int norm_type, int key_salt, bool head_done, const CycleWatch* decide) {
    int rc;
    const int nt = norm_type < 0 ? 9 : norm_type;
    constexpr bool mixed = sizeof(T) == 4;
    const bool foldable = !mixed && norm_type >= 0 && h->cfg.post_iters > 0 && h->cfg.smoother == GMG_SMOOTHER_MULTICOLOR_GS && !h->lv[0].ord.blocked;
    const int fold_type = foldable ? norm_type : -1;
    auto head = [&] { if (mixed) (void)hipMemsetAsync(h->lv[0].x32, 0, sizeof(float) * (size_t)h->lv[0].n_pad * d, h->stream); };
    auto tail = [&](int& err, int folded) {
        if (mixed) {
            const size_t cnt = (size_t)h->lv[0].n_pad * d;
            hipLaunchKernelGGL(gmgk::add_correction, dim3((unsigned)((cnt + 255) / 256)), dim3(256), 0, h->stream, h->lv[0].x32, h->lv[0].x, (int64_t)cnt);
            err = launch_residual_to_f32(h, d, norm_type);
        } else if (norm_type >= 0) err = launch_norm(h, d, norm_type, folded, decide);
        prof_mark(h);
    };
    if (h->coarse_device) {
        int err = GMG_OK;
        rc = run_graph(h, key_salt + G_FULL * 10000 + d * 10 + nt, [&] {
            head();
            enqueue_down<T>(h, d,  0,  false, head_done);
            enqueue_coarse_device<T>(h, d);
            tail(err, enqueue_up<T>(h, d, 0, fold_type));
        });
        return rc ? rc : err;
    }
    if ((rc = run_graph(h, key_salt + G_DOWN * 10000 + d * 10, [&] { head(); enqueue_down<T>(h, d,  0,  false, head_done); }))) return rc;
    if ((rc = coarse_host_begin<T>(h, d))) return rc;
    int err = GMG_OK;
    rc = run_graph(h, key_salt + G_UP * 10000 + d * 10 + nt, [&] { tail(err, enqueue_up<T>(h, d, 0, fold_type)); });
    const int served = coarse_host_serve(h);
    return rc ? rc : (served ? served : err);
}

int vcycle_resident(gmg_handle h, int d, int norm_type, bool head_done = false, const CycleWatch* decide = nullptr) {
    if (h->cfg.inner_precision) return vcycle_legs<float>(h, d, norm_type, 100000, head_done, decide);
    return vcycle_legs<double>(h, d, norm_type, 0, head_done, decide);
}


int ensure_accel(gmg_handle h) {
    auto& a = h->accel;
    const int m = h->cfg.accelerate, n_pad = h->lv[0].n_pad, D = h->dcap;
    if (a.xk && a.depth == m && a.d == D && a.n_pad == n_pad) return GMG_OK;
    a = {};
    const size_t count = (size_t)n_pad * D;
    auto vec = [&](DevBuf<double>* p) -> int {
        int rc = dev_alloc(h, *p, count);
        if (rc == GMG_OK) HIPCHK(hipMemsetAsync(*p, 0, sizeof(double) * count, h->stream));
        return rc;
    };
    int rc;
    for (DevBuf<double>* p : {&a.xk, &a.r, &a.z0}) if ((rc = vec(p))) return rc;
    for (int j = 0; j < m - 1; ++j) for (DevBuf<double>* p : {&a.zs[j], &a.qs[j]}) if ((rc = vec(p))) return rc;
    if ((rc = dev_alloc(h, a.scal, (size_t)9 * D + 1)) ||
        (rc = dev_alloc(h, a.partials, (size_t)gmgk::kAccelMaxBlocks * gmgk::kAccelMaxComp))) return rc;
    a.depth = m; a.d = D; a.n_pad = n_pad;
    return GMG_OK;
}

int launch_accel_step(gmg_handle h, int d, int type, int done) {
    auto& a = h->accel;
    Level& l = h->lv[0];
    const int DA = a.d, ld = l.n_pad, n_pairs = l.n_pad / 2, stored = a.depth - 1;
    const int ns = std::min(done, stored);
    const int wslot = stored > 0 ? done % stored : -1;
    const int nblk = std::max(1, std::min(gmgk::kAccelMaxBlocks, (n_pairs + gmgk::kAccelBlock - 1) / gmgk::kAccelBlock));
    const double* w = type == 1 ? h->d_minv : (type == 2 ? h->d_mass : nullptr);
    double *alpha = a.scal, *guarded = a.scal + DA, *beta = a.scal + 2 * DA, *s_slot = a.scal + 5 * DA, *guard_steps = a.scal + 8 * DA,
           *bb = a.scal + 8 * DA + 1;
    for_col_chunks(d, [&](int c0, int dc) {
        const size_t off = (size_t)c0 * ld;
        gmgk::AccelRing ring{};
        for (int j = 0; j < ns; ++j) { ring.z[j] = a.zs[j] + off; ring.q[j] = a.qs[j] + off; }
        double* q0 = l.r + off;
        double* zw = wslot >= 0 ? a.zs[wslot] + off : nullptr;
        double* qw = wslot >= 0 ? a.qs[wslot] + off : nullptr;
        DISPATCH_D(dc, hipLaunchKernelGGL((gmgk::accel_form<D>), dim3(nblk), dim3(gmgk::kAccelBlock), 0, h->stream, l.x + off, a.xk + off, a.r + off, q0, a.z0 + off,
                                          ring, ns, w, ld, n_pairs, a.partials));
        if (ns > 0)
            hipLaunchKernelGGL(gmgk::accel_reduce_beta, dim3(1), dim3(gmgk::kReduceBlock), 0, h->stream, a.partials, nblk, ns, dc, s_slot + c0, DA, beta + c0);
        DISPATCH_D(dc, hipLaunchKernelGGL((gmgk::accel_orth<D>), dim3(nblk), dim3(gmgk::kAccelBlock), 0, h->stream, a.z0 + off, q0, a.r + off, ring, ns, zw, qw,
                                          beta + c0, DA, w, ld, n_pairs, a.partials));
        hipLaunchKernelGGL(gmgk::accel_reduce_alpha, dim3(1), dim3(gmgk::kReduceBlock), 0, h->stream, a.partials, nblk, dc, alpha + c0, guarded + c0,
                           wslot >= 0 ? s_slot + (size_t)wslot * DA + c0 : nullptr, guard_steps, bb + c0);
        DISPATCH_D(dc, hipLaunchKernelGGL((gmgk::accel_update<D>), dim3(nblk), dim3(gmgk::kAccelBlock), 0, h->stream, a.xk + off, l.x + off, a.r + off,
                                          zw ? zw : a.z0 + off, qw ? qw : q0, a.z0 + off, q0, alpha + c0, guarded + c0, l.b + off, w, ld, n_pairs, a.partials));
        if (done == 0) hipLaunchKernelGGL(gmgk::accel_reduce_bb, dim3(1), dim3(gmgk::kReduceBlock), 0, h->stream, a.partials, nblk, dc, bb + c0);
        launch_reduce(h, nblk, dc, c0, c0 + 4 >= d, a.partials);
    });
    if (!polled(h)) HIPCHK(hipMemcpyAsync(h->h_norm, h->d_norm, sizeof(double) * 2 * d, hipMemcpyDeviceToHost, h->stream));
    return GMG_OK;
}

template <class Step>
int solve_loop(gmg_handle h, double tol, int max_iter, clk::time_point t0, double* conv, bool verbose, int* iters_out, double* residue_out, Step&& step) {
    SolveRule rule = rule_begin(tol, max_iter);
    bool go_on;
    do {
        double residue = 0.0; int device_go = -1;
        if (const int rc = step(rule, residue, device_go)) return rc;
        rule = rule_after(rule, residue);
        if (conv) { conv[2 * rule.cycles - 2] = ms_since(t0); conv[2 * rule.cycles - 1] = residue; }
        if (verbose) std::printf("%d,%f,%.14f \n", rule.cycles, ms_since(t0), residue);
        go_on = rule_goes_on(rule);
        if (device_go >= 0) {
            if ((device_go != 0) != go_on) h->timing["head_decision_differs"] += 1.0;
            go_on = device_go != 0;
        }
    } while (go_on);
    h->timing["cycles"] = ms_since(t0);
    const bool diverged = rule_diverged(rule);
    h->timing["diverged"] = diverged ? 1.0 : 0.0; h->timing["blown_up"] = rule.blown ? 1.0 : 0.0;
    h->timing["iterations"] = rule.cycles; h->timing["residue"] = rule.residue;
    if (iters_out) *iters_out = rule.cycles;
    if (residue_out) *residue_out = rule.residue;
    return diverged ? GMG_DIVERGED : GMG_OK;
}
// ... 20 lines not shown
```

### gravo_mg_amd/csrc/engine_state.hip.hpp

```cpp
#pragma once

inline std::shared_mutex& gate_mutex() { static std::shared_mutex* m = new std::shared_mutex(); return *m; }
static thread_local int tl_gates_held = 0;
struct DeviceSyncGuard {
    bool locked = false;
    DeviceSyncGuard() { if (tl_gates_held == 0) { gate_mutex().lock(); locked = true; } }
    ~DeviceSyncGuard() { if (locked) gate_mutex().unlock(); }
    DeviceSyncGuard(const DeviceSyncGuard&) = delete;
    DeviceSyncGuard& operator=(const DeviceSyncGuard&) = delete;
};
static inline hipError_t sync_hipFree(void* p) { DeviceSyncGuard g; return hipFree(p); }
static inline hipError_t sync_hipHostFree(void* p) { DeviceSyncGuard g; return hipHostFree(p); }
static inline hipError_t sync_hipStreamDestroy(hipStream_t s) { DeviceSyncGuard g; return hipStreamDestroy(s); }

struct DevPool {
    std::multimap<size_t, void*> parked;
    std::map<void*, size_t> size_of;
    size_t parked_bytes = 0, live_bytes = 0;
    size_t peak_live_bytes = 0;
    void reset_peak() { peak_live_bytes = live_bytes; }
    static size_t round_up(size_t b) { return (std::max<size_t>(b, 1) + 511) & ~(size_t)511; }
    hipError_t alloc(void** p, size_t bytes) {
        const size_t need = round_up(bytes);
        auto it = parked.lower_bound(need);
// ... 22 lines not shown
        parked.clear(); parked_bytes = 0;
    }
};
static thread_local DevPool* tl_pool = nullptr;
struct PoolScope {
    DevPool* prev;
    explicit PoolScope(DevPool* p) : prev(tl_pool) { tl_pool = p; }
    ~PoolScope() { tl_pool = prev; }
};
static inline hipError_t dev_malloc(void** p, size_t bytes) { return tl_pool ? tl_pool->alloc(p, bytes) : hipMalloc(p, bytes); }
static inline hipError_t dev_free(void* p) { if (!p) return hipSuccess; if (tl_pool) { tl_pool->release(p); return hipSuccess; } return sync_hipFree(p); }

#include "dev_buf.hpp"
inline void dev_buf_release(void* p) { (void)dev_free(p); }

namespace {

struct DevSell {
    int n_slices = 0;
    int lpr = 1;
    int64_t stored = 0, nnz_real = 0;
    DevBuf<int64_t> slice_ptr;
    DevBuf<int> col;
    DevBuf<double> val;
    DevBuf<float> val32;
    DevBuf<int> row_of;
    DevBuf<unsigned> col16;
    DevBuf<int> win_base;
    int c16_dbits = 13;
    int c16_mode = 0;
    int c16_from = 0;
    bool resident = false;
    int uniform_w = 0;
    int c16_arg() const { return (c16_mode == 1 ? c16_from : 0) | uniform_w << 24 | (c16_dbits == 11 ? 1 << 30 : 0); }
    int c16_sel() const { return c16_mode ? c16_mode + (resident ? 2 : 0) : 0; }
};

struct DevCsr {
    int n_outer = 0;
    DevBuf<int> ptr, idx;
    DevBuf<double> val;
};

struct DevEll3 {
    int n = 0;
    DevBuf<int> cnt, col;
    DevBuf<double> val;
};

struct Level {
    int n = 0, n_pad = 0;
    int64_t nnz = 0;
    LevelOrdering ord;
    Compressed A;
    bool hostA_pattern = false, hostA_values = false;
    DevCsr dA;
    DevSell Aoff;
    DevBuf<double> diag;
    double cheby_lambda = 0.0;
    DevSell P, R;
    DevSell Ain, Aout;
    DevBuf<unsigned short> ain_col16;
    bool use_bcsr = false;
    DevBuf<int> bc_ptr, bc_mid, bc_col;
    DevBuf<double> bc_val;
    DevBuf<float> bc_val32;
    int bc_cap = 0;
    int64_t bc_nnz = 0;
    bool use_ep = false;
    DevBuf<int> ee_ptr, ee_col, ep_ptr;
    DevBuf<unsigned short> ep_col;
    DevBuf<double> ee_val, ep_val;
    DevBuf<float> ee_val32, ep_val32;
    int64_t ee_nnz = 0, ep_nnz = 0;
    int ep_cap_e = 0, ep_cap_l = 0;
    DevBuf<int> d_blk_begin, d_blk_ncolors;
    DevBuf<unsigned char> d_row_color;
    DevBuf<int> src_A, src_diag, src_ee, src_ep;
    DevBuf<int> d_new2old;
    DevBuf<int> d_old2new;
    DevBuf<int> d_blk_of_row;
    DevBuf<double> x, b, r, tmp;
    DevBuf<float> diag32, x32, b32, r32, tmp32;
};

}

struct FineGraph {
    int n = 0;
    RawVec<int> ptr, idx;
};

struct gmg_hierarchy_s {
    HierarchyResult res;
    std::shared_ptr<const FineGraph> graph;
    std::vector<int> fine_order;
};

struct DistP2P;

struct DistPlan {
    int rank = 0, world = 1, n_colors = 0;
    bool shard1 = false;
    uint64_t key[2] = {0, 0};
    std::vector<int> blk_owner;
    std::vector<std::vector<int>> own_blocks;
    std::vector<std::vector<int>> halo;
    std::vector<std::vector<int>> halo1, halo0r;
};

enum class LiveSystem { none, placeholder, system };

struct gmg_solver_s {
    DevPool pool;
    DistP2P* p2p = nullptr;
    double dbg_cheby_ratio = 0.0;
    int dbg_col16_uncovered = 0;
    gmg_config cfg;
    std::string err;
    bool has_device = false;
    int n_cus = 256;
    hipStream_t stream = nullptr;
    int L = -1;
    std::vector<Compressed> U;
    std::vector<char> U_set;
    std::vector<DevCsr> dU;
    std::vector<DevEll3> dE3;
    bool dU_ready = false;
    std::vector<PatchSet> patches;
    std::vector<int> cluster_order;
    DevBuf<int> d_cluster_order, d_cluster_inv;
    std::vector<int> bfs_order;
    std::shared_ptr<const FineGraph> fine_graph;
    bool mass_dirty = false;
    DevBuf<int> d_bfs_order, d_bfs_inv;
    int base_order_choice = 0;
    RawVec<int> reo_ptr, reo_idx;
    bool patches_ready = false;
    bool dU_flagged = false;
    std::vector<double> mass;
    std::vector<Level> lv;
    SupernodalLDLT coarse;
    LiveSystem live = LiveSystem::none;
    int dcap = 0;
    DevBuf<double> d_mass, d_minv;
    DevBuf<double> d_stage; size_t stage_cap = 0;
    double* h_stage[2] = {nullptr, nullptr}; size_t h_stage_cap = 0;
    void* bounce[2] = {nullptr, nullptr};
    hipEvent_t bounce_ev[2] = {nullptr, nullptr}; int bounce_flip = 0;
    hipEvent_t h_stage_ev[2] = {nullptr, nullptr}; int h_stage_flip = 0;
    hipEvent_t h_chunk_ev[16] = {};
    DevBuf<double> d_partials; int partial_blocks = 0;
    DevBuf<double> d_norm;
    struct AccelState {
        DevBuf<double> xk, r, z0;
        DevBuf<double> zs[gmg::kAccelMaxStored];
        DevBuf<double> qs[gmg::kAccelMaxStored];
        DevBuf<double> scal;
        DevBuf<double> partials;
        int depth = 0, d = 0, n_pad = 0;
    } accel;
    DevBuf<double> d_watch;
    double* h_pinned = nullptr; size_t pinned_cap = 0;
    double* h_norm = nullptr;
    unsigned long long* h_flag = nullptr; unsigned long long flag_seq[3] = {0, 0, 0};
    bool gate_ok = true;
// ... 286 lines not shown
```

### gravo_mg_amd/csrc/kernels.hip.hpp

```cpp
#pragma once
#include <hip/hip_runtime.h>
#include <stdint.h>
#include "solve_rule.hpp"
#include "coarse_triangle.hpp"

namespace gmgk {

constexpr int kBlock = 256;
constexpr int kWavesPerBlock = kBlock / 64;

__device__ __forceinline__ int wave_slice(int n_slices_total, int xcd_swizzle) {
    int nblk = gridDim.x;
    int b = blockIdx.x;
    if (xcd_swizzle && (nblk & 7) == 0) b = (b & 7) * (nblk >> 3) + (b >> 3);
    int w = b * kWavesPerBlock + (threadIdx.x >> 6);
    (void)n_slices_total;
    return __builtin_amdgcn_readfirstlane(w);
}

template <int D, int XI> __device__ __forceinline__ int64_t x_at(int c, int d, int ld) { return XI ? (int64_t)c * D + d : c + (int64_t)d * ld; }

__device__ __forceinline__ float fma_of(float a, float b, float c) { return __builtin_fmaf(a, b, c); }
__device__ __forceinline__ double fma_of(double a, double b, double c) { return __builtin_fma(a, b, c); }

template <class T, int D, int W, int XI = 0>
__device__ __forceinline__ void row_dot_group(const int* __restrict__ cp, const T* __restrict__ vp, const T* x, int ld,
                                              T (&acc)[D]) {
    int c[W];
    T v[W];
#pragma unroll
    for (int j = 0; j < W; ++j) { c[j] = __builtin_nontemporal_load(cp + j * 64); v[j] = __builtin_nontemporal_load(vp + j * 64); }
    T xv[W][D];
#pragma unroll
    for (int j = 0; j < W; ++j)
#pragma unroll
        for (int d = 0; d < D; ++d) xv[j][d] = x[x_at<D, XI>(c[j], d, ld)];
#pragma unroll
    for (int j = 0; j < W; ++j)
#pragma unroll
        for (int d = 0; d < D; ++d) acc[d] = fma_of(v[j], xv[j][d], acc[d]);
}

template <int D> struct DotGroup { static constexpr int value = D >= 4 ? 4 : (D == 3 ? 6 : 8); };
template <class T, int D, int G = DotGroup<D>::value, int XI = 0>
__device__ __forceinline__ void row_dot(const int64_t* __restrict__ slice_ptr, const int* __restrict__ col,
                                        const T* __restrict__ val, const T* x, int ld, int s, int lane,
                                        T (&acc)[D], int uw = 0) {
    const int64_t p0 = uw ? (int64_t)s * (uw << 6) : slice_ptr[s];
    int w = uw ? uw : (int)((slice_ptr[s + 1] - p0) >> 6);
    const int* cp = col + p0 + lane;
    const T* vp = val + p0 + lane;
#pragma unroll
    for (int c = 0; c < D; ++c) acc[c] = 0.0;
    for (; w >= G; w -= G, cp += G * 64, vp += G * 64) row_dot_group<T, D, G, XI>(cp, vp, x, ld, acc);
    switch (w) {
        case 1: row_dot_group<T, D, 1, XI>(cp, vp, x, ld, acc); break;
        case 2: row_dot_group<T, D, 2, XI>(cp, vp, x, ld, acc); break;
        case 3: row_dot_group<T, D, 3, XI>(cp, vp, x, ld, acc); break;
        case 4: if (G > 4) row_dot_group<T, D, 4, XI>(cp, vp, x, ld, acc); break;
        case 5: if (G > 4) row_dot_group<T, D, 5, XI>(cp, vp, x, ld, acc); break;
        case 6: if (G > 4) row_dot_group<T, D, 6, XI>(cp, vp, x, ld, acc); break;
        case 7: if (G > 4) row_dot_group<T, D, 7, XI>(cp, vp, x, ld, acc); break;
        default: break;
    }
}

template <class T, int D, int W, bool FLAGS, int XI = 0, bool KEEP = false>
__device__ __forceinline__ void row_dot_group16(const unsigned* __restrict__ cp, const int* __restrict__ cp32, const T* __restrict__ vp, const T* x, int ld,
                                                int basev, int dbits, int& fallback, T (&acc)[D]) {
    unsigned pk[(W + 1) / 2];
    T v[W];
#pragma unroll
    for (int q = 0; q < (W + 1) / 2; ++q) pk[q] = KEEP ? cp[q * 64] : __builtin_nontemporal_load(cp + q * 64);
#pragma unroll
    for (int j = 0; j < W; ++j) v[j] = KEEP ? vp[j * 64] : __builtin_nontemporal_load(vp + j * 64);
    if constexpr (FLAGS) { if (fallback < 0) fallback = __builtin_amdgcn_readfirstlane(basev) < 0 ? 1 : 0; }
    int c[W];
    if (FLAGS && fallback) {
#pragma unroll
        for (int j = 0; j < W; ++j) c[j] = __builtin_nontemporal_load(cp32 + j * 64);
    } else {
        const unsigned mask = (1u << dbits) - 1u;
#pragma unroll
        for (int j = 0; j < W; ++j) {
            const unsigned u = (j & 1) ? pk[j >> 1] >> 16 : pk[j >> 1] & 0xffffu;
            c[j] = __builtin_amdgcn_ds_bpermute((int)((u >> dbits) << 2), basev) + (int)(u & mask);
        }
    }
    T xv[W][D];
#pragma unroll
    for (int j = 0; j < W; ++j)
#pragma unroll
        for (int d = 0; d < D; ++d) xv[j][d] = x[x_at<D, XI>(c[j], d, ld)];
#pragma unroll
    for (int j = 0; j < W; ++j)
#pragma unroll
        for (int d = 0; d < D; ++d) acc[d] = fma_of(v[j], xv[j][d], acc[d]);
}

template <class T, int D, bool FLAGS, int G = DotGroup<D>::value, int XI = 0, bool KEEP = false>
__device__ __forceinline__ void row_dot16(const int64_t* __restrict__ slice_ptr, const int* __restrict__ col, const unsigned* __restrict__ col16,
                                          const int* __restrict__ win_base, int dbits, const T* __restrict__ val, const T* x, int ld, int s, int lane, T (&acc)[D], int uw = 0) {
    const int wshift = 16 - dbits;
    const int basev = win_base[((int64_t)s << wshift) + (lane & ((1 << wshift) - 1))];
    const int64_t p0 = uw ? (int64_t)s * (uw << 6) : slice_ptr[s];
    int w = uw ? uw : (int)((slice_ptr[s + 1] - p0) >> 6);
    const unsigned* cp = col16 + p0 + lane;
    const int* cp32 = col + p0 + lane;
    const T* vp = val + p0 + lane;
    int fallback = -1;
#pragma unroll
    for (int c = 0; c < D; ++c) acc[c] = 0.0;
    for (; w >= G; w -= G, cp += (G / 2) * 64, cp32 += G * 64, vp += G * 64) row_dot_group16<T, D, G, FLAGS, XI, KEEP>(cp, cp32, vp, x, ld, basev, dbits, fallback, acc);
    switch (w) {
        case 1: row_dot_group16<T, D, 1, FLAGS, XI, KEEP>(cp, cp32, vp, x, ld, basev, dbits, fallback, acc); break;
        case 2: row_dot_group16<T, D, 2, FLAGS, XI, KEEP>(cp, cp32, vp, x, ld, basev, dbits, fallback, acc); break;
        case 3: row_dot_group16<T, D, 3, FLAGS, XI, KEEP>(cp, cp32, vp, x, ld, basev, dbits, fallback, acc); break;
        case 4: if (G > 4) row_dot_group16<T, D, 4, FLAGS, XI, KEEP>(cp, cp32, vp, x, ld, basev, dbits, fallback, acc); break;
        case 5: if (G > 4) row_dot_group16<T, D, 5, FLAGS, XI, KEEP>(cp, cp32, vp, x, ld, basev, dbits, fallback, acc); break;
        case 6: if (G > 4) row_dot_group16<T, D, 6, FLAGS, XI, KEEP>(cp, cp32, vp, x, ld, basev, dbits, fallback, acc); break;
        case 7: if (G > 4) row_dot_group16<T, D, 7, FLAGS, XI, KEEP>(cp, cp32, vp, x, ld, basev, dbits, fallback, acc); break;
        default: break;
    }
}

template <class T, int D, int C16, int G = DotGroup<D>::value, int XI = 0>
__device__ __forceinline__ void row_dot_sel(const int64_t* __restrict__ slice_ptr, const int* __restrict__ col, const unsigned* __restrict__ col16,
                                            const int* __restrict__ win_base, int c16_arg, const T* __restrict__ val, const T* x, int ld, int s, int lane,
                                            T (&acc)[D]) {
    if constexpr (C16 == 1 || C16 == 3) {
        const int dbits = (c16_arg >> 30) & 1 ? 11 : 13;
        const int uw = (c16_arg >> 24) & 63;
        if (s >= (c16_arg & 0xffffff)) row_dot16<T, D, false, G, XI, C16 == 3>(slice_ptr, col, col16, win_base, dbits, val, x, ld, s, lane, acc, uw);
        else row_dot<T, D, G, XI>(slice_ptr, col, val, x, ld, s, lane, acc, uw);
    } else if constexpr (C16 == 2 || C16 == 4) {
        row_dot16<T, D, true, G, XI, C16 == 4>(slice_ptr, col, col16, win_base, (c16_arg >> 30) & 1 ? 11 : 13, val, x, ld, s, lane, acc, (c16_arg >> 24) & 63);
    } else row_dot<T, D, G, XI>(slice_ptr, col, val, x, ld, s, lane, acc);
}

template <class T, int D>
__device__ __forceinline__ void quad_reduce(T (&acc)[D]) {
#pragma unroll
    for (int c = 0; c < D; ++c) {
        acc[c] += __shfl_xor(acc[c], 1, 64);
        acc[c] += __shfl_xor(acc[c], 2, 64);
    }
}

template <class T> __device__ __forceinline__ T gs_row(T bi, T acc, T dg) { return (bi - acc) / dg; }
template <class T> __device__ __forceinline__ T gs_row(T bi, T acc, T dg, T omega, T xi) { return xi + omega * (gs_row(bi, acc, dg) - xi); }

template <class T> __device__ __forceinline__ T row_ax(T acc, T dg, T xi) { return acc + dg * xi; }
__device__ __forceinline__ double norm_term(double v, double w) { return (v * w) * v; }
template <int NW, int D, class SLOT>
__device__ __forceinline__ void block_sums_store(const double (&sums)[2 * D], double (&red)[NW][2 * D], int wave, int lane, SLOT slot, double* __restrict__ partials) {
#pragma unroll
    for (int c = 0; c < 2 * D; ++c) {
        double v = sums[c];
#pragma unroll
        for (int off = 32; off > 0; off >>= 1) v += __shfl_down(v, off, 64);
        if (lane == 0) red[wave][c] = v;
    }
    __syncthreads();
    if (threadIdx.x < 2 * D) {
        double v = 0.0;
#pragma unroll
        for (int w2 = 0; w2 < NW; ++w2) v += red[w2][threadIdx.x];
        partials[(int64_t)slot * (2 * D) + threadIdx.x] = v;
    }
}

template <class T, int D, int FINE, int OM = 0>
__global__ __launch_bounds__(kBlock) void gs_color(const int64_t* __restrict__ slice_ptr, const int* __restrict__ col,
                                                   const T* __restrict__ val, const T* __restrict__ diag,
                                                   const T* __restrict__ b, T* x, int ld, int slice_begin,
                                                   int slice_end, int xcd_swizzle, T omega, const unsigned* __restrict__ col16 = nullptr,
                                                   const int* __restrict__ win_base = nullptr, int c16_arg = 0,
                                                   const unsigned long long* __restrict__ plain_rows = nullptr, const int* __restrict__ go = nullptr) {
    if (go != nullptr && *go == 0) return;
    const int s = slice_begin + wave_slice(slice_end - slice_begin, xcd_swizzle);
    if (s >= slice_end) return;
    const int lane = threadIdx.x & 63;
    const int row = s * 64 + lane;
    T acc[D];
    row_dot_sel<T, D, (FINE >= 2 ? FINE - 1 : 0)>(slice_ptr, col, col16, win_base, c16_arg, val, x, ld, s, lane, acc);
    const T dg = diag[row];
    if constexpr (OM != 0) {
        const T om = (plain_rows[s] >> lane) & 1ull ? (T)1.0 : omega;
#pragma unroll
        for (int c = 0; c < D; ++c) {
            const T xi = x[row + (int64_t)c * ld];
            x[row + (int64_t)c * ld] = gs_row(b[row + (int64_t)c * ld], acc[c], dg, om, xi);
        }
        return;
    }
    if (omega == (T)1.0) {
#pragma unroll
        for (int c = 0; c < D; ++c) x[row + (int64_t)c * ld] = gs_row(b[row + (int64_t)c * ld], acc[c], dg);
    } else {
#pragma unroll
        for (int c = 0; c < D; ++c) {
            const T xi = x[row + (int64_t)c * ld];
            x[row + (int64_t)c * ld] = gs_row(b[row + (int64_t)c * ld], acc[c], dg, omega, xi);
        }
    }
}

template <int D, int C16 = 0>
__global__ __launch_bounds__(kBlock) void gs_color_norm(const int64_t* __restrict__ slice_ptr, const int* __restrict__ col,
                                                        const double* __restrict__ val, const double* __restrict__ diag,
                                                        const double* __restrict__ b, double* x, int ld, int slice_begin, int slice_end,
                                                        double omega, const double* __restrict__ weight, double* __restrict__ partials,
                                                        const unsigned* __restrict__ col16 = nullptr, const int* __restrict__ win_base = nullptr, int c16_arg = 0) {
    __shared__ double red[kWavesPerBlock][2 * D];
    const int s = slice_begin + wave_slice(slice_end - slice_begin, 1);
    const int wave = threadIdx.x >> 6, lane = threadIdx.x & 63;
    double sums[2 * D];
#pragma unroll
    for (int c = 0; c < 2 * D; ++c) sums[c] = 0.0;
    if (s < slice_end) {
        const int row = s * 64 + lane;
        double acc[D];
        row_dot_sel<double, D, C16>(slice_ptr, col, col16, win_base, c16_arg, val, x, ld, s, lane, acc);
        const double dg = diag[row];
        const double w = weight ? weight[row] : 1.0;
#pragma unroll
        for (int c = 0; c < D; ++c) {
            const double bi = b[row + (int64_t)c * ld];
            const double xi = x[row + (int64_t)c * ld];
            const double xn = omega == 1.0 ? gs_row(bi, acc[c], dg) : gs_row(bi, acc[c], dg, omega, xi);
            x[row + (int64_t)c * ld] = xn;
            const double r = row_ax(acc[c], dg, xn) - bi;
            sums[2 * c] = norm_term(r, w);
            sums[2 * c + 1] = norm_term(bi, w);
        }
    }
    block_sums_store<kWavesPerBlock, D>(sums, red, wave, lane, (unsigned)blockIdx.x, partials);
}

template <int D, int C16 = 0, int YI = 0>
__global__ __launch_bounds__(kBlock) void gs_color_residual(const int64_t* __restrict__ slice_ptr, const int* __restrict__ col,
                                                            const double* __restrict__ val, const double* __restrict__ diag,
                                                            const double* __restrict__ b, double* x, double* __restrict__ r, int ld,
                                                            int slice_begin, int slice_end, double omega, const unsigned* __restrict__ col16 = nullptr,
                                                            const int* __restrict__ win_base = nullptr, int c16_arg = 0) {
    const int s = slice_begin + wave_slice(slice_end - slice_begin, 1);
    if (s >= slice_end) return;
    const int lane = threadIdx.x & 63;
    const int row = s * 64 + lane;
    double acc[D];
    row_dot_sel<double, D, C16>(slice_ptr, col, col16, win_base, c16_arg, val, x, ld, s, lane, acc);
    const double dg = diag[row];
#pragma unroll
    for (int c = 0; c < D; ++c) {
        const double bi = b[row + (int64_t)c * ld];
        double xn;
        if (omega == 1.0) xn = gs_row(bi, acc[c], dg);
        else { const double xi = x[row + (int64_t)c * ld]; xn = gs_row(bi, acc[c], dg, omega, xi); }
        x[row + (int64_t)c * ld] = xn;
        const double ax = row_ax(acc[c], dg, xn);
        r[YI ? (int64_t)row * D + c : row + (int64_t)c * ld] = bi - ax;
    }
}

constexpr int kBlockRows = 1024;
template <class T, int D, int WIN>
__global__ __launch_bounds__(kBlockRows) void gs_block(const int* __restrict__ blk_begin, const int* __restrict__ blk_ncolors,
                                                       const unsigned char* __restrict__ row_color,
                                                       const int64_t* __restrict__ in_ptr, const unsigned short* __restrict__ in_col,
                                                       const T* __restrict__ in_val, const int64_t* __restrict__ out_ptr,
                                                       const int* __restrict__ out_col, const T* __restrict__ out_val,
                                                       const T* __restrict__ diag, const T* __restrict__ b,
                                                       const T* __restrict__ x_in, T* __restrict__ x_out, int ld) {
    __shared__ T xs[D][kBlockRows];
    const int blk = blockIdx.x;
    const int r0 = blk_begin[blk];
    const int nrows = blk_begin[blk + 1] - r0;
    const int t = threadIdx.x, lane = t & 63;
    const int wave = __builtin_amdgcn_readfirstlane(t >> 6);
    const bool active = wave * 64 < nrows;
    const int row = r0 + t;
    T rhs[D], dg = 1.0;
    int mycolor = -1, w = 0;
    int64_t p0 = 0;
#pragma unroll
// ... 1087 lines not shown
__global__ __launch_bounds__(kBlock) void fetch_from_host(const double* src, double* __restrict__ dst, int n) {
    const unsigned long long* s = reinterpret_cast<const unsigned long long*>(src);
    for (int i = blockIdx.x * kBlock + threadIdx.x; i < n; i += gridDim.x * kBlock)
        dst[i] = __longlong_as_double((long long)__hip_atomic_load(s + i, __ATOMIC_RELAXED, __HIP_MEMORY_SCOPE_SYSTEM));
}

template <int D>
__global__ __launch_bounds__(kBlock) void residual_norm_partials(const int64_t* __restrict__ slice_ptr, const int* __restrict__ col,
                                                                 const double* __restrict__ val, const double* __restrict__ diag,
                                                                 const double* __restrict__ b, const double* __restrict__ x,
                                                                 const double* __restrict__ weight, int ld, int slice_begin,
                                                                 int slice_end, double* __restrict__ partials) {
    __shared__ double red[kWavesPerBlock][2 * D];
    const int wave = threadIdx.x >> 6, lane = threadIdx.x & 63;
    double sums[2 * D];
#pragma unroll
    for (int c = 0; c < 2 * D; ++c) sums[c] = 0.0;
    for (int s = slice_begin + __builtin_amdgcn_readfirstlane(blockIdx.x * kWavesPerBlock + wave); s < slice_end;
         s += gridDim.x * kWavesPerBlock) {
        const int row = s * 64 + lane;
        double acc[D];
        row_dot<double, D>(slice_ptr, col, val, x, ld, s, lane, acc);
        const double dg = diag[row];
        const double w = weight ? weight[row] : 1.0;
#pragma unroll
        for (int c = 0; c < D; ++c) {
            const double bi = b[row + (int64_t)c * ld];
            const double r = row_ax(acc[c], dg, x[row + (int64_t)c * ld]) - bi;
            sums[2 * c] += norm_term(r, w);
            sums[2 * c + 1] += norm_term(bi, w);
        }
    }
#pragma unroll
    for (int c = 0; c < 2 * D; ++c) {
        double v = sums[c];
#pragma unroll
        for (int off = 32; off > 0; off >>= 1) v += __shfl_down(v, off, 64);
        if (lane == 0) red[wave][c] = v;
    }
    __syncthreads();
    if (threadIdx.x < 2 * D) {
        double v = 0.0;
#pragma unroll
        for (int w2 = 0; w2 < kWavesPerBlock; ++w2) v += red[w2][threadIdx.x];
        partials[(int64_t)blockIdx.x * (2 * D) + threadIdx.x] = v;
    }
}

constexpr int kNormWaves = 16;
template <int D, int MODE, int C16 = 0>
__global__ __launch_bounds__(kNormWaves * 64, 8) void residual_norm_slices(const int64_t* __restrict__ slice_ptr, const int* __restrict__ col,
                                                               const double* __restrict__ val, const double* __restrict__ diag,
                                                               const double* __restrict__ b, const double* __restrict__ x,
                                                               const double* __restrict__ weight, int ld, int n_slices,
                                                               float* __restrict__ r32, double* __restrict__ partials,
                                                               const unsigned* __restrict__ col16 = nullptr, const int* __restrict__ win_base = nullptr, int c16_arg = 0) {
    __shared__ double red[kNormWaves][2 * D];
    const int wave = threadIdx.x >> 6, lane = threadIdx.x & 63;
    int nblk = gridDim.x, bb = blockIdx.x;
    if ((nblk & 7) == 0) bb = (bb & 7) * (nblk >> 3) + (bb >> 3);
    const int s = __builtin_amdgcn_readfirstlane(bb * kNormWaves + wave);
    double sums[2 * D];
#pragma unroll
    for (int c = 0; c < 2 * D; ++c) sums[c] = 0.0;
    if (s < n_slices) {
        const int row = s * 64 + lane;
        double acc[D];
        row_dot_sel<double, D, C16>(slice_ptr, col, col16, win_base, c16_arg, val, x, ld, s, lane, acc);
        const double dg = diag[row];
        const double w = weight ? weight[row] : 1.0;
#pragma unroll
        for (int c = 0; c < D; ++c) {
            const double bi = b[row + (int64_t)c * ld];
            double r;
            if (MODE == 1) { r = bi - row_ax(acc[c], dg, x[row + (int64_t)c * ld]); r32[row + (int64_t)c * ld] = (float)r; }
            else r = row_ax(acc[c], dg, x[row + (int64_t)c * ld]) - bi;
            sums[2 * c] = norm_term(r, w);
            sums[2 * c + 1] = norm_term(bi, w);
        }
    }
    block_sums_store<kNormWaves, D>(sums, red, wave, lane, bb, partials);
}

__global__ void add_correction(const float* __restrict__ e, double* __restrict__ x, int64_t n) {
    const int64_t i = (int64_t)blockIdx.x * blockDim.x + threadIdx.x;
    if (i < n) x[i] += (double)e[i];
}

__global__ void cvt_f64_to_f32(const double* __restrict__ src, float* __restrict__ dst, int64_t n) {
    const int64_t i = (int64_t)blockIdx.x * blockDim.x + threadIdx.x;
    if (i < n) dst[i] = (float)src[i];
}

__global__ void cvt_f32_to_f64(const float* __restrict__ src, double* __restrict__ dst, int64_t n) {
    const int64_t i = (int64_t)blockIdx.x * blockDim.x + threadIdx.x;
    if (i < n) dst[i] = (double)src[i];
}

__global__ void permute_in(const double* __restrict__ src, int n, const int* __restrict__ new2old, double* __restrict__ dst,
                           int ld, int n_pad, int D) {
    const int r = blockIdx.x * blockDim.x + threadIdx.x;
    if (r >= n_pad) return;
    const int old = new2old[r];
    for (int c = 0; c < D; ++c) dst[r + (int64_t)c * ld] = old >= 0 ? src[old + (int64_t)c * n] : 0.0;
}

__global__ void permute_out(const double* __restrict__ src, int ld, int n_pad, const int* __restrict__ new2old,
                            double* __restrict__ dst, int n, int D) {
    const int r = blockIdx.x * blockDim.x + threadIdx.x;
    if (r >= n_pad) return;
    const int old = new2old[r];
    if (old < 0) return;
    for (int c = 0; c < D; ++c) dst[old + (int64_t)c * n] = src[r + (int64_t)c * ld];
}

template <int D, bool X0>
__global__ __launch_bounds__(256) void permute_in2_strided(const double* rhs, int64_t rhs_rs, int64_t rhs_cs, const double* x0, int64_t x0_rs, int64_t x0_cs,
                                                           const int* __restrict__ new2old, double* __restrict__ b, double* __restrict__ x, int ld,
                                                           int n_pad, int d) {
    const int r = blockIdx.x * blockDim.x + threadIdx.x;
    if (r >= n_pad) return;
    const int old = new2old[r];
    const double* pb = rhs + (int64_t)(old >= 0 ? old : 0) * rhs_rs;
    const double* px = X0 ? x0 + (int64_t)(old >= 0 ? old : 0) * x0_rs : nullptr;
    if (D > 0) {
        double vb[D > 0 ? D : 1], vx[D > 0 ? D : 1];
#pragma unroll
        for (int c = 0; c < D; ++c) {
            vb[c] = old >= 0 ? pb[(int64_t)c * rhs_cs] : 0.0;
            vx[c] = X0 ? (old >= 0 ? px[(int64_t)c * x0_cs] : 0.0) : vb[c];
        }
#pragma unroll
        for (int c = 0; c < D; ++c) { b[r + (int64_t)c * ld] = vb[c]; x[r + (int64_t)c * ld] = vx[c]; }
    } else {
        for (int c = 0; c < d; ++c) {
            const double vb = old >= 0 ? pb[(int64_t)c * rhs_cs] : 0.0;
            const double vx = X0 ? (old >= 0 ? px[(int64_t)c * x0_cs] : 0.0) : vb;
            b[r + (int64_t)c * ld] = vb;
            x[r + (int64_t)c * ld] = vx;
        }
    }
}

template <int D>
__global__ __launch_bounds__(256) void permute_out_strided(const double* __restrict__ src, int ld, int n_pad, const int* __restrict__ new2old,
                                                           double* __restrict__ dst, int64_t dst_rs, int64_t dst_cs, int d) {
    const int r = blockIdx.x * blockDim.x + threadIdx.x;
    if (r >= n_pad) return;
    const int old = new2old[r];
    if (old < 0) return;
    double* p = dst + (int64_t)old * dst_rs;
    if (D > 0) {
        double v[D > 0 ? D : 1];
#pragma unroll
        for (int c = 0; c < D; ++c) v[c] = src[r + (int64_t)c * ld];
#pragma unroll
        for (int c = 0; c < D; ++c) p[(int64_t)c * dst_cs] = v[c];
    } else {
        for (int c = 0; c < d; ++c) p[(int64_t)c * dst_cs] = src[r + (int64_t)c * ld];
    }
}

__global__ __launch_bounds__(256) void stieltjes_signs_flag(int n, const int* __restrict__ ptr, const int* __restrict__ idx, const double* __restrict__ val,
                                                            int* __restrict__ flag) {
    const int j = blockIdx.x * blockDim.x + threadIdx.x;
    if (j >= n) return;
// ... 267 lines not shown
```

### include/gravomg_hip.h

```cpp
#ifndef GRAVOMG_HIP_H
#define GRAVOMG_HIP_H

#include <stdint.h>

#ifdef __cplusplus
extern "C" {
#endif

typedef struct gmg_solver_s* gmg_handle;
typedef struct gmg_hierarchy_s* gmg_hierarchy;

typedef enum {
    GMG_OK = 0,
    GMG_ERR_INVALID = -1,
    GMG_ERR_NO_DEVICE = -2,
    GMG_ERR_HIP = -3,
    GMG_ERR_STATE = -4,
    GMG_ERR_NUMERIC = -5,
    GMG_ERR_UNSUPPORTED = -6,
    GMG_DIVERGED = 1
} gmg_status;

enum { GMG_SMOOTHER_MULTICOLOR_GS = 0, GMG_SMOOTHER_JACOBI = 1, GMG_SMOOTHER_CHEBYSHEV = 2 };
enum { GMG_COARSE_HOST_LDLT = 0, GMG_COARSE_DEVICE_INVERSE = 1, GMG_COARSE_AUTO = 2, GMG_COARSE_DEVICE_TRIANGLE = 3 };

typedef struct {
    int device;
    int smoother;
    double jacobi_omega;
    int pre_iters;
    int post_iters;
    int coarse_mode;
    int use_graph;
    int sigma;
    int row_align;
    int block_rows;
    int block_lanes;
    int block_from_level;
    int device_setup;
    int device_rap;
    int reorder_fine;
    int inner_precision;
    int block_csr;
    int host_threads;
    int verbose;
    double gs_omega;
    int restrict_sigma;
    int block_ep;
    int dist_shard_levels;
    int block_fine;
    int fine_col16;
    int stream_gate;
    int dist_exchange;
    int prepare_structure;
    int fuse_restrict_sweep;
    int speculate_head;
    int uniform_slices;
    int color_ahead;
    int accelerate;
} gmg_config;

int gmg_config_default(gmg_config* cfg);
int gmg_config_size(void);
int gmg_create(const gmg_config* cfg, gmg_handle* out);
void gmg_destroy(gmg_handle h);
const char* gmg_last_error(gmg_handle h);
int gmg_host_threads(void);
int gmg_device_count(void);

int gmg_set_num_levels(gmg_handle h, int L);
int gmg_set_prolongation(gmg_handle h, int k, int n_fine, int n_coarse, const int* colptr, const int* rowidx, const double* val);
int gmg_set_mass(gmg_handle h, int n, const double* mass_diag);
int gmg_set_system(gmg_handle h, int n, const int* colptr, const int* rowidx, const double* val);
int gmg_set_system_values_device(gmg_handle h, const double* d_val, int64_t nnz);

int gmg_num_levels(gmg_handle h);
int gmg_level_info(gmg_handle h, int k, int* n, int64_t* nnz, int* n_colors, int* n_pad);
int gmg_get_level_operator(gmg_handle h, int k, int* colptr, int* rowidx, double* val);
int gmg_get_level_ordering(gmg_handle h, int k, int* new2old, int* color_begin);
int gmg_get_level_blocks(gmg_handle h, int k, int* n_blocks, int* blk_begin, unsigned char* row_color);
int gmg_get_timing(gmg_handle h, const char* key, double* out);

int gmg_smooth(gmg_handle h, int k, const double* b, double* x, int d, int iters);
int gmg_smooth_residual(gmg_handle h, int k, const double* b, double* x, int d, int iters, int from_zero, double* r);
int gmg_residual(gmg_handle h, int k, const double* b, const double* x, int d, double* r);
int gmg_spmv(gmg_handle h, int k, const double* x, int d, double* y);
int gmg_restrict(gmg_handle h, int k, const double* r, int d, double* rc);
int gmg_prolong_add(gmg_handle h, int k, const double* e, int d, double* x);
int gmg_coarse_solve(gmg_handle h, const double* rc, int d, double* e);
int gmg_residual_norm(gmg_handle h, const double* b, const double* x, int d, int type, double* out);

int gmg_vcycle(gmg_handle h, const double* b, double* x, int d);
int gmg_solve(gmg_handle h, const double* rhs, double* x, int d, double tol, int stop_type, int max_iter,
              int* iters_out, double* residue_out, double* conv);
int gmg_solve_x0_rhs(gmg_handle h, const double* rhs, double* x, int d, double tol, int stop_type, int max_iter,
                     int* iters_out, double* residue_out, double* conv);
typedef struct {
    const double* rhs;  int64_t rhs_row_stride, rhs_col_stride;
    const double* x0;   int64_t x0_row_stride,  x0_col_stride;
    double*       x;    int64_t x_row_stride,   x_col_stride;
} gmg_device_vectors;
int gmg_solve_device(gmg_handle h, const gmg_device_vectors* v, int d, double tol, int stop_type, int max_iter,
                     int* iters_out, double* residue_out, double* conv);

int gmg_load_problem(gmg_handle h, const double* b, const double* x0, int d);
int gmg_run_cycles(gmg_handle h, int n_cycles, int stop_type, double* residues);
int gmg_fetch_solution(gmg_handle h, double* x);

int gmg_set_stream(gmg_handle h, void* hip_stream);
int gmg_dist_setup(gmg_handle h, int rank, int world);
int gmg_dist_partition(gmg_handle h, int rank, int world);
int gmg_dist_bind(gmg_handle h, double* x0, double* b0, double* r0, int d);
int gmg_dist_smooth_color(gmg_handle h, int c);
int gmg_dist_residual_own(gmg_handle h);
int gmg_dist_coarse_cycle(gmg_handle h);
int gmg_dist_prolong_own(gmg_handle h);
int gmg_dist_norm_partial(gmg_handle h, int type, double* sums);
int gmg_dist_all_rows(gmg_handle h, int on);
int gmg_dist_gather(gmg_handle h, const double* src, const int64_t* idx, int64_t n, double* dst);
int gmg_dist_scatter(gmg_handle h, const double* src, const int64_t* pos, const int64_t* idx, int64_t n, double* dst);

int gmg_p2p_blob_bytes(void);
int gmg_p2p_prepare(gmg_handle h, int rank, int world, int d);
int gmg_p2p_export(gmg_handle h, void* blob_out);
int gmg_p2p_connect(gmg_handle h, const void* blobs);
int gmg_p2p_rccl_unique_id(void* id_out_128_bytes);
int gmg_p2p_connect_rccl(gmg_handle h, const void* id_128_bytes);
int gmg_p2p_load(gmg_handle h, const double* b, const double* x0);
int gmg_p2p_cycles(gmg_handle h, int n_cycles, int stop_type, double* residues);
int gmg_p2p_fetch(gmg_handle h, double* x);
int gmg_p2p_solve(gmg_handle h, const double* b, double* x, double tol, int stop_type, int max_iter, int* iters_out, double* residue_out);
int gmg_p2p_stat(gmg_handle h, const char* key, double* out);
int gmg_p2p_set_smoother(gmg_handle h, int mode);
int gmg_p2p_set_fences(gmg_handle h, int fenced);

typedef struct {
    double ratio;
    int lower_bound;
    int check_voronoi;
    int nested;
    int sampling;
// ... 32 lines not shown
```

Measured before the change: 0.5789.

## Fold speculative first-color GS head into residual-norm kernel and commit with second color

When the residual check runs, the residual-norm kernel now also computes the next cycle's first-color Gauss-Seidel update into a side buffer. A new commit kernel then sweeps the second color using those shadow values and copies the buffer into x, so the separate head color launch goes away. The goal is to remove one kernel launch and one pass over the fine matrix per V-cycle. In exchange it adds an extra buffer, an alternate-row indirection in the gather, and more complex speculation state. It is enabled by default.

Result: faster. 0.5722 (median of 6 runs) (-1.2%).

```diff
diff --git a/gravo_mg_amd/cabi.py b/gravo_mg_amd/cabi.py
--- a/gravo_mg_amd/cabi.py
+++ b/gravo_mg_amd/cabi.py
@@ -34,7 +34,7 @@
         ("row_align", C.c_int), ("block_rows", C.c_int), ("block_lanes", C.c_int), ("block_from_level", C.c_int),
         ("device_setup", C.c_int), ("device_rap", C.c_int), ("reorder_fine", C.c_int), ("inner_precision", C.c_int), ("block_csr", C.c_int), ("host_threads", C.c_int),
         ("verbose", C.c_int), ("gs_omega", C.c_double), ("restrict_sigma", C.c_int), ("block_ep", C.c_int), ("dist_shard_levels", C.c_int), ("block_fine", C.c_int), ("fine_col16", C.c_int), ("stream_gate", C.c_int), ("dist_exchange", C.c_int), ("prepare_structure", C.c_int), ("fuse_restrict_sweep", C.c_int), ("speculate_head", C.c_int), ("uniform_slices", C.c_int), ("color_ahead", C.c_int),
-        ("accelerate", C.c_int),
+        ("fold_head", C.c_int), ("accelerate", C.c_int),
     ]
 
 
@@ -319,7 +319,7 @@
 
     def __init__(self, smoother=SMOOTHER_MULTICOLOR_GS, pre_iters=2, post_iters=2, jacobi_omega=0.67,
                  coarse_mode=COARSE_AUTO, use_graph=False, sigma=0, row_align=64, block_rows=64, block_from_level=1, block_lanes=0,
-                 device_setup=True, device_rap=True, reorder_fine=2, inner_precision=0, block_csr=True, device=0, verbose=False, gs_omega=None, block_ep=None, restrict_sigma=None, dist_shard_levels=None, block_fine=None, fine_col16=None, stream_gate=None, prepare_structure=None, dist_exchange=None, fuse_restrict_sweep=None, speculate_head=None, uniform_slices=None, color_ahead=None, accelerate=0):
+                 device_setup=True, device_rap=True, reorder_fine=2, inner_precision=0, block_csr=True, device=0, verbose=False, gs_omega=None, block_ep=None, restrict_sigma=None, dist_shard_levels=None, block_fine=None, fine_col16=None, stream_gate=None, prepare_structure=None, dist_exchange=None, fuse_restrict_sweep=None, speculate_head=None, uniform_slices=None, color_ahead=None, accelerate=0, fold_head=None):
         l = lib()
         cfg = GmgConfig()
         l.gmg_config_default(C.byref(cfg))
@@ -356,6 +356,8 @@
         if dist_exchange is not None:
             cfg.dist_exchange = int(dist_exchange)
         cfg.accelerate = int(accelerate)
+        if fold_head is not None:
+            cfg.fold_head = int(bool(fold_head))
         self._h = _vp()
         rc = l.gmg_create(C.byref(cfg), C.byref(self._h))
         if rc:
diff --git a/gravo_mg_amd/csrc/bindings.cpp b/gravo_mg_amd/csrc/bindings.cpp
--- a/gravo_mg_amd/csrc/bindings.cpp
+++ b/gravo_mg_amd/csrc/bindings.cpp
@@ -308,6 +308,7 @@
         else if (key == "dist_exchange") c.dist_exchange = (int)value;
         else if (key == "inner_precision") c.inner_precision = (int)value;
         else if (key == "accelerate") c.accelerate = (int)value;
+        else if (key == "fold_head") c.fold_head = (int)value;
         else throw std::invalid_argument("unknown engine option: " + key);
     }
 
diff --git a/gravo_mg_amd/csrc/engine.hip b/gravo_mg_amd/csrc/engine.hip
--- a/gravo_mg_amd/csrc/engine.hip
+++ b/gravo_mg_amd/csrc/engine.hip
@@ -114,6 +114,7 @@
     cfg->prepare_structure = 1;
     cfg->fuse_restrict_sweep = 1;
     cfg->speculate_head = 1;
+    cfg->fold_head = 1;
     cfg->uniform_slices = 1;
     cfg->color_ahead = 1;
     cfg->dist_exchange = 0;
@@ -580,7 +581,7 @@
 namespace {
 inline bool loop_enqueues_heads(gmg_handle h, int d, bool wanted) {
     if (!wanted || !head_eligible(h, d)) return false;
-    h->timing["heads_enqueued"] += 0.0; h->timing["head_decision_differs"] += 0.0;
+    h->timing["heads_enqueued"] += 0.0; h->timing["head_decision_differs"] += 0.0; h->timing["heads_folded"] += 0.0;
     return true;
 }
 }
@@ -596,12 +597,14 @@
     HelperScope helper_scope(h, d);
     const bool heads = loop_enqueues_heads(h, d, stop_type >= 0);
     CycleWatch watch{0, 0.0, stop_type, 0};
-    bool head_done = false;
+    int head_done = HEAD_NONE;
     for (int i = 0; i < n_cycles; ++i) {
         watch.cycles_done = i + 1;
+        const bool head = heads && i + 1 < n_cycles;
+        watch.fold = head && fold_eligible(h, d);
         if ((rc = vcycle_resident(h, d, stop_type, head_done, heads ? &watch : nullptr))) return rc;
         if (stop_type >= 0) {
-            head_done = heads && i + 1 < n_cycles && enqueue_head(h, d);
+            head_done = head ? enqueue_head(h, d, watch.fold) : HEAD_NONE;
             if ((rc = wait_norm(h))) return rc;
             if (residues) residues[i] = norm_from_sums(h->h_norm, d, stop_type);
         }
@@ -689,16 +692,17 @@
     };
     const bool heads = loop_enqueues_heads(h, d, accel == 0);
     CycleWatch watch{1, tol, stop_type, 0};
-    bool head_done = false;
+    int head_done = HEAD_NONE;
     auto plain_step = [&](const SolveRule& rule, double& residue, int& device_go) -> int {
         watch.cycles_done = rule.cycles + 1;
         const bool head = heads && rule.cycles + 2 <= rule.max_iter;
+        watch.fold = head && fold_eligible(h, d);
         if ((rc = vcycle_resident(h, d, stop_type, head_done, heads ? &watch : nullptr))) return rc;
-        head_done = head && enqueue_head(h, d);
+        head_done = head ? enqueue_head(h, d, watch.fold) : HEAD_NONE;
         if ((rc = wait_norm(h))) return rc;
         residue = norm_from_sums(h->h_norm, d, stop_type);
         if (head) device_go = __atomic_load_n(h->h_flag + 1, __ATOMIC_ACQUIRE) != 0;
-        if (device_go == 0) head_done = false;
+        if (device_go == 0) head_done = HEAD_NONE;
         return GMG_OK;
     };
     int verdict;
diff --git a/gravo_mg_amd/csrc/engine_cycle.hip.hpp b/gravo_mg_amd/csrc/engine_cycle.hip.hpp
--- a/gravo_mg_amd/csrc/engine_cycle.hip.hpp
+++ b/gravo_mg_amd/csrc/engine_cycle.hip.hpp
@@ -59,7 +59,7 @@
 struct SmoothAsk {
     bool from_zero = false;
     bool first_done = false;
-    bool head_done = false;
+    int head_done = 0;
     T* res_out = nullptr;
     bool res_il = false;
     int norm_type = -1;
@@ -131,24 +131,48 @@
            !h->lv[0].ord.blocked && h->lv[0].ord.n_colors >= 2 && first_color(h->lv[0]) >= 0 && first_color(h->lv[0]) < h->lv[0].ord.n_colors - 1 && d >= 1 && d <= 4 &&
            !h->partitioned && h->part_world <= 1 && h->d_watch && !h->prof_on;
 }
-inline bool enqueue_head(gmg_handle h, int d) {
+inline int second_color(const Level& l) {
+    for (int c = first_color(l) + 1; c > 0 && c < l.ord.n_colors; ++c)
+        if (l.ord.color_begin[c + 1] / 64 > l.ord.color_begin[c] / 64) return c;
+    return -1;
+}
+inline bool fold_eligible(gmg_handle h, int d) {
+    if (!h->cfg.fold_head || h->cfg.accelerate != 0 || !head_eligible(h, d)) return false;
+    const Level& l = h->lv[0];
+    const int c1 = first_color(l), c2 = second_color(l);
+    return c2 > 0 && (c2 < l.ord.n_colors - 1 || h->cfg.pre_iters >= 2) && l.xh &&
+           l.xh_rows == (l.ord.color_begin[c1 + 1] / 64 - l.ord.color_begin[c1] / 64) * 64 && d <= h->dcap;
+}
+enum { HEAD_NONE = 0, HEAD_FIRST = 1, HEAD_FOLDED = 2 };
+inline int enqueue_head(gmg_handle h, int d, bool folded = false) {
     Level& l = h->lv[0];
     const int c = first_color(l);
-    launch_gs_color<double>(h, l, 0, d, l.ord.color_begin[c] / 64, l.ord.color_begin[c + 1] / 64, level_omega<double>(h, l), nullptr, reinterpret_cast<const int*>(h->d_watch + 1));
+    const int* go = reinterpret_cast<const int*>(h->d_watch + 1);
     h->timing["heads_enqueued"] += 1.0;
-    return true;
+    if (!folded) {
+        launch_gs_color<double>(h, l, 0, d, l.ord.color_begin[c] / 64, l.ord.color_begin[c + 1] / 64, level_omega<double>(h, l), nullptr, go);
+        return HEAD_FIRST;
+    }
+    const int c2 = second_color(l);
+    const int hb = l.ord.color_begin[c] / 64, he = l.ord.color_begin[c + 1] / 64, sb = l.ord.color_begin[c2] / 64, se = l.ord.color_begin[c2 + 1] / 64;
+    const int n_work = grid_for(se - sb), n_copy = ((he - hb) * 32 + gmgk::kBlock - 1) / gmgk::kBlock;
+    DISPATCH_D(d, DISPATCH_C16(l.Aoff.c16_sel(), hipLaunchKernelGGL((gmgk::gs_color_commit<D, C16>), dim3(n_work + n_copy), dim3(gmgk::kBlock), 0, h->stream,
+                                     l.Aoff.slice_ptr, l.Aoff.col, l.Aoff.val, l.diag, l.b, l.x, l.n_pad, sb, se, n_work, level_omega<double>(h, l), l.Aoff.col16,
+                                     l.Aoff.win_base, l.Aoff.c16_arg(), l.xh.get(), hb, he, go)));
+    h->timing["heads_folded"] += 1.0;
+    return HEAD_FOLDED;
 }
 
 template <class T>
 SmoothDone<T> launch_gs_sweeps(gmg_handle h, Level& l, int d, int iters, const SmoothAsk<T>& ask) {
     SmoothDone<T> done;
-    const int c_head = ask.head_done ? first_color(l) : -1;
+    const int c_head = ask.head_done ? first_color(l) : -1, c_head2 = ask.head_done == HEAD_FOLDED ? second_color(l) : -1;
     for (int it = 0; it < iters; ++it)
         for_col_chunks(d, [&](int c0, int dc) {
             for (int c = 0; c < l.ord.n_colors; ++c) {
                 int sb = l.ord.color_begin[c] / 64, se = l.ord.color_begin[c + 1] / 64;
                 if (se <= sb) continue;
-                if (it == 0 && c0 == 0 && c == c_head) continue;
+                if (it == 0 && c0 == 0 && (c == c_head || c == c_head2)) continue;
                 const bool last_launch = it == iters - 1 && c == l.ord.n_colors - 1;
                 if (const int nblk = fold_norm<T>(h, l, d, last_launch, sb, se, ask.norm_type)) { done.norm_blocks = nblk; continue; }
                 if (const int from = fold_residual<T>(h, l, d, last_launch, sb, se, ask.res_out, ask.res_il)) { done.res_from = from; continue; }
@@ -418,7 +442,7 @@
     return GMG_OK;
 }
 
-struct CycleWatch { int mode; double tol; int type; int cycles_done; };
+struct CycleWatch { int mode; double tol; int type; int cycles_done; bool fold = false; };
 
 void launch_reduce(gmg_handle h, int nblk, int dc, int c0, bool last, const double* partials = nullptr, const CycleWatch* decide = nullptr) {
     if (!partials) partials = h->d_partials;
@@ -440,10 +464,18 @@
     const int n_slices = folded ? l.ord.color_begin[l.ord.n_colors - 1] / 64 : l.Aoff.n_slices;
     const int nblk = norm_grid(n_slices);
     const bool poll = polled(h);
-    for_col_chunks(d, [&](int c0, int dc) {
-        DISPATCH_D(dc, DISPATCH_C16(l.Aoff.c16_sel(), hipLaunchKernelGGL((gmgk::residual_norm_slices<D, 0, C16>), dim3(nblk), dim3(gmgk::kNormWaves * 64), 0, h->stream,
-                                          l.Aoff.slice_ptr, l.Aoff.col, l.Aoff.val, l.diag, l.b + (size_t)c0 * l.n_pad, l.x + (size_t)c0 * l.n_pad, w,
-                                          l.n_pad, n_slices, (float*)nullptr, h->d_partials, l.Aoff.col16, l.Aoff.win_base, l.Aoff.c16_arg())));
+    const int c_head = decide && decide->fold && d <= 4 ? first_color(l) : -1;
+    for_col_chunks(d, [&](int c0, int dc) {
+        if (c_head >= 0) {
+            DISPATCH_D(dc, DISPATCH_C16(l.Aoff.c16_sel(), hipLaunchKernelGGL((gmgk::residual_norm_slices_head<D, C16>), dim3(nblk), dim3(gmgk::kNormWaves * 64), 0, h->stream,
+                                              l.Aoff.slice_ptr, l.Aoff.col, l.Aoff.val, l.diag, l.b.get(), l.x.get(), w, l.n_pad, n_slices, h->d_partials.get(), l.Aoff.col16,
+                                              l.Aoff.win_base, l.Aoff.c16_arg(), l.xh.get(), l.ord.color_begin[c_head] / 64, l.ord.color_begin[c_head + 1] / 64,
+                                              level_omega<double>(h, l))));
+        } else {
+            DISPATCH_D(dc, DISPATCH_C16(l.Aoff.c16_sel(), hipLaunchKernelGGL((gmgk::residual_norm_slices<D, 0, C16>), dim3(nblk), dim3(gmgk::kNormWaves * 64), 0, h->stream,
+                                              l.Aoff.slice_ptr, l.Aoff.col, l.Aoff.val, l.diag, l.b + (size_t)c0 * l.n_pad, l.x + (size_t)c0 * l.n_pad, w,
+                                              l.n_pad, n_slices, (float*)nullptr, h->d_partials, l.Aoff.col16, l.Aoff.win_base, l.Aoff.c16_arg())));
+        }
         launch_reduce(h, nblk + folded, dc, c0, c0 + 4 >= d, nullptr, decide);
     });
     if (!poll) HIPCHK(hipMemcpyAsync(h->h_norm, h->d_norm, sizeof(double) * 2 * d, hipMemcpyDeviceToHost, h->stream));
@@ -468,6 +500,17 @@
         int rc;
         if ((rc = vec(l.x, l, true)) || (rc = vec(l.b, l, true)) || (rc = vec(l.r, l, true)) || (rc = vec(l.tmp, l, tmp)) ||
             (rc = vec(l.x32, l, f32)) || (rc = vec(l.b32, l, f32)) || (rc = vec(l.r32, l, f32)) || (rc = vec(l.tmp32, l, f32 && tmp))) return rc;
+    }
+    {
+        Level& l0 = h->lv[0];
+        const int fc = h->cfg.fold_head && !l0.ord.blocked ? first_color(l0) : -1;
+        l0.xh.reset(); l0.xh_rows = 0;
+        if (fc >= 0) {
+            const int rows = (l0.ord.color_begin[fc + 1] / 64 - l0.ord.color_begin[fc] / 64) * 64;
+            int rc = dev_alloc(h, l0.xh, (size_t)rows * d);
+            if (rc) return rc;
+            l0.xh_rows = rows;
+        }
     }
     Level& c = h->lv[h->L];
     size_t need = (size_t)c.n_pad * d * 2;
@@ -655,7 +698,7 @@
 }
 
 template <class T = double>
-void enqueue_down(gmg_handle h, int d, int k0 = 0, bool first_done = false, bool head_done = false) {
+void enqueue_down(gmg_handle h, int d, int k0 = 0, bool first_done = false, int head_done = 0) {
     const int L = h->L;
     for (int k = k0; k < L; ++k) {
         Level& l = h->lv[k];
@@ -663,7 +706,7 @@
         SmoothAsk<T> ask;
         ask.from_zero = k > 0 && smooth_from_zero_ok(h, l, h->cfg.pre_iters);
         if (k > 0 && !ask.from_zero) (void)hipMemsetAsync(Prec<T>::x(l), 0, sizeof(T) * (size_t)l.n_pad * d, h->stream);
-        ask.first_done = first_done; ask.head_done = k == 0 && head_done;
+        ask.first_done = first_done; ask.head_done = k == 0 ? head_done : 0;
         const bool il = k == 0 && d > 1 && d <= 4 && l.Aoff.lpr == 1;
         if (k == 0 && sizeof(T) == 8) { ask.res_out = Prec<T>::r(l); ask.res_il = il; }
         const SmoothDone<T> swept = launch_smooth<T>(h, l, d, h->cfg.pre_iters, ask);
@@ -892,7 +935,7 @@
 }
 
 template <class T>
-int vcycle_legs(gmg_handle h, int d, int norm_type, int key_salt, bool head_done, const CycleWatch* decide) {
+int vcycle_legs(gmg_handle h, int d, int norm_type, int key_salt, int head_done, const CycleWatch* decide) {
     int rc;
     const int nt = norm_type < 0 ? 9 : norm_type;
     constexpr bool mixed = sizeof(T) == 4;
@@ -925,7 +968,7 @@
     return rc ? rc : (served ? served : err);
 }
 
-int vcycle_resident(gmg_handle h, int d, int norm_type, bool head_done = false, const CycleWatch* decide = nullptr) {
+int vcycle_resident(gmg_handle h, int d, int norm_type, int head_done = 0, const CycleWatch* decide = nullptr) {
     if (h->cfg.inner_precision) return vcycle_legs<float>(h, d, norm_type, 100000, head_done, decide);
     return vcycle_legs<double>(h, d, norm_type, 0, head_done, decide);
 }
diff --git a/gravo_mg_amd/csrc/engine_state.hip.hpp b/gravo_mg_amd/csrc/engine_state.hip.hpp
--- a/gravo_mg_amd/csrc/engine_state.hip.hpp
+++ b/gravo_mg_amd/csrc/engine_state.hip.hpp
@@ -128,6 +128,8 @@
     DevBuf<int> d_blk_of_row;
     DevBuf<double> x, b, r, tmp;
     DevBuf<float> diag32, x32, b32, r32, tmp32;
+    DevBuf<double> xh;
+    int xh_rows = 0;
 };
 
 }
diff --git a/gravo_mg_amd/csrc/kernels.hip.hpp b/gravo_mg_amd/csrc/kernels.hip.hpp
--- a/gravo_mg_amd/csrc/kernels.hip.hpp
+++ b/gravo_mg_amd/csrc/kernels.hip.hpp
@@ -23,9 +23,18 @@
 __device__ __forceinline__ float fma_of(float a, float b, float c) { return __builtin_fmaf(a, b, c); }
 __device__ __forceinline__ double fma_of(double a, double b, double c) { return __builtin_fma(a, b, c); }
 
-template <class T, int D, int W, int XI = 0>
+template <class T> struct AltRows { const T* shifted = nullptr; unsigned lo = 0, n = 0; };
+template <class T, int D>
+__device__ __forceinline__ T alt_at(const AltRows<T>& alt, const T* x, int c, int d, int ld) {
+    const bool in = (unsigned)c - alt.lo < alt.n;
+    const T* p = in ? alt.shifted : x;
+    if (D == 1) return p[c];
+    return p[c + (int64_t)d * (in ? (int)alt.n : ld)];
+}
+
+template <class T, int D, int W, int XI = 0, bool ALT = false>
 __device__ __forceinline__ void row_dot_group(const int* __restrict__ cp, const T* __restrict__ vp, const T* x, int ld,
-                                              T (&acc)[D]) {
+                                              T (&acc)[D], const AltRows<T>& alt = AltRows<T>{}) {
     int c[W];
     T v[W];
 #pragma unroll
@@ -34,7 +43,7 @@
 #pragma unroll
     for (int j = 0; j < W; ++j)
 #pragma unroll
-        for (int d = 0; d < D; ++d) xv[j][d] = x[x_at<D, XI>(c[j], d, ld)];
+        for (int d = 0; d < D; ++d) xv[j][d] = ALT ? alt_at<T, D>(alt, x, c[j], d, ld) : x[x_at<D, XI>(c[j], d, ld)];
 #pragma unroll
     for (int j = 0; j < W; ++j)
 #pragma unroll
@@ -42,32 +51,32 @@
 }
 
 template <int D> struct DotGroup { static constexpr int value = D >= 4 ? 4 : (D == 3 ? 6 : 8); };
-template <class T, int D, int G = DotGroup<D>::value, int XI = 0>
+template <class T, int D, int G = DotGroup<D>::value, int XI = 0, bool ALT = false>
 __device__ __forceinline__ void row_dot(const int64_t* __restrict__ slice_ptr, const int* __restrict__ col,
                                         const T* __restrict__ val, const T* x, int ld, int s, int lane,
-                                        T (&acc)[D], int uw = 0) {
+                                        T (&acc)[D], int uw = 0, const AltRows<T>& alt = AltRows<T>{}) {
     const int64_t p0 = uw ? (int64_t)s * (uw << 6) : slice_ptr[s];
     int w = uw ? uw : (int)((slice_ptr[s + 1] - p0) >> 6);
     const int* cp = col + p0 + lane;
     const T* vp = val + p0 + lane;
 #pragma unroll
     for (int c = 0; c < D; ++c) acc[c] = 0.0;
-    for (; w >= G; w -= G, cp += G * 64, vp += G * 64) row_dot_group<T, D, G, XI>(cp, vp, x, ld, acc);
+    for (; w >= G; w -= G, cp += G * 64, vp += G * 64) row_dot_group<T, D, G, XI, ALT>(cp, vp, x, ld, acc, alt);
     switch (w) {
-        case 1: row_dot_group<T, D, 1, XI>(cp, vp, x, ld, acc); break;
-        case 2: row_dot_group<T, D, 2, XI>(cp, vp, x, ld, acc); break;
-        case 3: row_dot_group<T, D, 3, XI>(cp, vp, x, ld, acc); break;
-        case 4: if (G > 4) row_dot_group<T, D, 4, XI>(cp, vp, x, ld, acc); break;
-        case 5: if (G > 4) row_dot_group<T, D, 5, XI>(cp, vp, x, ld, acc); break;
-        case 6: if (G > 4) row_dot_group<T, D, 6, XI>(cp, vp, x, ld, acc); break;
-        case 7: if (G > 4) row_dot_group<T, D, 7, XI>(cp, vp, x, ld, acc); break;
+        case 1: row_dot_group<T, D, 1, XI, ALT>(cp, vp, x, ld, acc, alt); break;
+        case 2: row_dot_group<T, D, 2, XI, ALT>(cp, vp, x, ld, acc, alt); break;
+        case 3: row_dot_group<T, D, 3, XI, ALT>(cp, vp, x, ld, acc, alt); break;
+        case 4: if (G > 4) row_dot_group<T, D, 4, XI, ALT>(cp, vp, x, ld, acc, alt); break;
+        case 5: if (G > 4) row_dot_group<T, D, 5, XI, ALT>(cp, vp, x, ld, acc, alt); break;
+        case 6: if (G > 4) row_dot_group<T, D, 6, XI, ALT>(cp, vp, x, ld, acc, alt); break;
+        case 7: if (G > 4) row_dot_group<T, D, 7, XI, ALT>(cp, vp, x, ld, acc, alt); break;
         default: break;
     }
 }
 
-template <class T, int D, int W, bool FLAGS, int XI = 0, bool KEEP = false>
+template <class T, int D, int W, bool FLAGS, int XI = 0, bool KEEP = false, bool ALT = false>
 __device__ __forceinline__ void row_dot_group16(const unsigned* __restrict__ cp, const int* __restrict__ cp32, const T* __restrict__ vp, const T* x, int ld,
-                                                int basev, int dbits, int& fallback, T (&acc)[D]) {
+                                                int basev, int dbits, int& fallback, T (&acc)[D], const AltRows<T>& alt = AltRows<T>{}) {
     unsigned pk[(W + 1) / 2];
     T v[W];
 #pragma unroll
@@ -91,16 +100,17 @@
 #pragma unroll
     for (int j = 0; j < W; ++j)
 #pragma unroll
-        for (int d = 0; d < D; ++d) xv[j][d] = x[x_at<D, XI>(c[j], d, ld)];
+        for (int d = 0; d < D; ++d) xv[j][d] = ALT ? alt_at<T, D>(alt, x, c[j], d, ld) : x[x_at<D, XI>(c[j], d, ld)];
 #pragma unroll
     for (int j = 0; j < W; ++j)
 #pragma unroll
         for (int d = 0; d < D; ++d) acc[d] = fma_of(v[j], xv[j][d], acc[d]);
 }
 
-template <class T, int D, bool FLAGS, int G = DotGroup<D>::value, int XI = 0, bool KEEP = false>
+template <class T, int D, bool FLAGS, int G = DotGroup<D>::value, int XI = 0, bool KEEP = false, bool ALT = false>
 __device__ __forceinline__ void row_dot16(const int64_t* __restrict__ slice_ptr, const int* __restrict__ col, const unsigned* __restrict__ col16,
-                                          const int* __restrict__ win_base, int dbits, const T* __restrict__ val, const T* x, int ld, int s, int lane, T (&acc)[D], int uw = 0) {
+                                          const int* __restrict__ win_base, int dbits, const T* __restrict__ val, const T* x, int ld, int s, int lane, T (&acc)[D], int uw = 0,
+                                          const AltRows<T>& alt = AltRows<T>{}) {
     const int wshift = 16 - dbits;
     const int basev = win_base[((int64_t)s << wshift) + (lane & ((1 << wshift) - 1))];
     const int64_t p0 = uw ? (int64_t)s * (uw << 6) : slice_ptr[s];
@@ -111,31 +121,31 @@
     int fallback = -1;
 #pragma unroll
     for (int c = 0; c < D; ++c) acc[c] = 0.0;
-    for (; w >= G; w -= G, cp += (G / 2) * 64, cp32 += G * 64, vp += G * 64) row_dot_group16<T, D, G, FLAGS, XI, KEEP>(cp, cp32, vp, x, ld, basev, dbits, fallback, acc);
+    for (; w >= G; w -= G, cp += (G / 2) * 64, cp32 += G * 64, vp += G * 64) row_dot_group16<T, D, G, FLAGS, XI, KEEP, ALT>(cp, cp32, vp, x, ld, basev, dbits, fallback, acc, alt);
     switch (w) {
-        case 1: row_dot_group16<T, D, 1, FLAGS, XI, KEEP>(cp, cp32, vp, x, ld, basev, dbits, fallback, acc); break;
-        case 2: row_dot_group16<T, D, 2, FLAGS, XI, KEEP>(cp, cp32, vp, x, ld, basev, dbits, fallback, acc); break;
-        case 3: row_dot_group16<T, D, 3, FLAGS, XI, KEEP>(cp, cp32, vp, x, ld, basev, dbits, fallback, acc); break;
-        case 4: if (G > 4) row_dot_group16<T, D, 4, FLAGS, XI, KEEP>(cp, cp32, vp, x, ld, basev, dbits, fallback, acc); break;
-        case 5: if (G > 4) row_dot_group16<T, D, 5, FLAGS, XI, KEEP>(cp, cp32, vp, x, ld, basev, dbits, fallback, acc); break;
-        case 6: if (G > 4) row_dot_group16<T, D, 6, FLAGS, XI, KEEP>(cp, cp32, vp, x, ld, basev, dbits, fallback, acc); break;
-        case 7: if (G > 4) row_dot_group16<T, D, 7, FLAGS, XI, KEEP>(cp, cp32, vp, x, ld, basev, dbits, fallback, acc); break;
+        case 1: row_dot_group16<T, D, 1, FLAGS, XI, KEEP, ALT>(cp, cp32, vp, x, ld, basev, dbits, fallback, acc, alt); break;
+        case 2: row_dot_group16<T, D, 2, FLAGS, XI, KEEP, ALT>(cp, cp32, vp, x, ld, basev, dbits, fallback, acc, alt); break;
+        case 3: row_dot_group16<T, D, 3, FLAGS, XI, KEEP, ALT>(cp, cp32, vp, x, ld, basev, dbits, fallback, acc, alt); break;
+        case 4: if (G > 4) row_dot_group16<T, D, 4, FLAGS, XI, KEEP, ALT>(cp, cp32, vp, x, ld, basev, dbits, fallback, acc, alt); break;
+        case 5: if (G > 4) row_dot_group16<T, D, 5, FLAGS, XI, KEEP, ALT>(cp, cp32, vp, x, ld, basev, dbits, fallback, acc, alt); break;
+        case 6: if (G > 4) row_dot_group16<T, D, 6, FLAGS, XI, KEEP, ALT>(cp, cp32, vp, x, ld, basev, dbits, fallback, acc, alt); break;
+        case 7: if (G > 4) row_dot_group16<T, D, 7, FLAGS, XI, KEEP, ALT>(cp, cp32, vp, x, ld, basev, dbits, fallback, acc, alt); break;
         default: break;
     }
 }
 
-template <class T, int D, int C16, int G = DotGroup<D>::value, int XI = 0>
+template <class T, int D, int C16, int G = DotGroup<D>::value, int XI = 0, bool ALT = false>
 __device__ __forceinline__ void row_dot_sel(const int64_t* __restrict__ slice_ptr, const int* __restrict__ col, const unsigned* __restrict__ col16,
                                             const int* __restrict__ win_base, int c16_arg, const T* __restrict__ val, const T* x, int ld, int s, int lane,
-                                            T (&acc)[D]) {
+                                            T (&acc)[D], const AltRows<T>& alt = AltRows<T>{}) {
     if constexpr (C16 == 1 || C16 == 3) {
         const int dbits = (c16_arg >> 30) & 1 ? 11 : 13;
         const int uw = (c16_arg >> 24) & 63;
-        if (s >= (c16_arg & 0xffffff)) row_dot16<T, D, false, G, XI, C16 == 3>(slice_ptr, col, col16, win_base, dbits, val, x, ld, s, lane, acc, uw);
-        else row_dot<T, D, G, XI>(slice_ptr, col, val, x, ld, s, lane, acc, uw);
+        if (s >= (c16_arg & 0xffffff)) row_dot16<T, D, false, G, XI, C16 == 3, ALT>(slice_ptr, col, col16, win_base, dbits, val, x, ld, s, lane, acc, uw, alt);
+        else row_dot<T, D, G, XI, ALT>(slice_ptr, col, val, x, ld, s, lane, acc, uw, alt);
     } else if constexpr (C16 == 2 || C16 == 4) {
-        row_dot16<T, D, true, G, XI, C16 == 4>(slice_ptr, col, col16, win_base, (c16_arg >> 30) & 1 ? 11 : 13, val, x, ld, s, lane, acc, (c16_arg >> 24) & 63);
-    } else row_dot<T, D, G, XI>(slice_ptr, col, val, x, ld, s, lane, acc);
+        row_dot16<T, D, true, G, XI, C16 == 4, ALT>(slice_ptr, col, col16, win_base, (c16_arg >> 30) & 1 ? 11 : 13, val, x, ld, s, lane, acc, (c16_arg >> 24) & 63, alt);
+    } else row_dot<T, D, G, XI, ALT>(slice_ptr, col, val, x, ld, s, lane, acc, 0, alt);
 }
 
 template <class T, int D>
@@ -201,6 +211,45 @@
 #pragma unroll
         for (int c = 0; c < D; ++c) {
             const T xi = x[row + (int64_t)c * ld];
+            x[row + (int64_t)c * ld] = gs_row(b[row + (int64_t)c * ld], acc[c], dg, omega, xi);
+        }
+    }
+}
+
+template <int D, int C16>
+__global__ __launch_bounds__(kBlock) void gs_color_commit(const int64_t* __restrict__ slice_ptr, const int* __restrict__ col,
+                                                          const double* __restrict__ val, const double* __restrict__ diag,
+                                                          const double* __restrict__ b, double* x, int ld, int slice_begin, int slice_end,
+                                                          int n_work, double omega, const unsigned* __restrict__ col16, const int* __restrict__ win_base,
+                                                          int c16_arg, const double* __restrict__ xh, int hb, int he, const int* __restrict__ go) {
+    if (*go == 0) return;
+    const int lane = threadIdx.x & 63;
+    const int hrows = (he - hb) * 64;
+    if ((int)blockIdx.x >= n_work) {
+        const int r = (((int)blockIdx.x - n_work) * kBlock + (int)threadIdx.x) * 2;
+        if (r >= hrows) return;
+#pragma unroll
+        for (int c = 0; c < D; ++c)
+            *reinterpret_cast<double2*>(x + (int64_t)hb * 64 + r + (int64_t)c * ld) = *reinterpret_cast<const double2*>(xh + r + (int64_t)c * hrows);
+        return;
+    }
+    int bb = blockIdx.x;
+    if ((n_work & 7) == 0) bb = (bb & 7) * (n_work >> 3) + (bb >> 3);
+    const int s = slice_begin + __builtin_amdgcn_readfirstlane(bb * kWavesPerBlock + (int)(threadIdx.x >> 6));
+    if (s >= slice_end) return;
+    const int row = s * 64 + lane;
+    AltRows<double> alt;
+    alt.shifted = xh - (int64_t)hb * 64; alt.lo = (unsigned)hb * 64u; alt.n = (unsigned)hrows;
+    double acc[D];
+    row_dot_sel<double, D, C16, DotGroup<D>::value, 0, true>(slice_ptr, col, col16, win_base, c16_arg, val, x, ld, s, lane, acc, alt);
+    const double dg = diag[row];
+    if (omega == 1.0) {
+#pragma unroll
+        for (int c = 0; c < D; ++c) x[row + (int64_t)c * ld] = gs_row(b[row + (int64_t)c * ld], acc[c], dg);
+    } else {
+#pragma unroll
+        for (int c = 0; c < D; ++c) {
+            const double xi = x[row + (int64_t)c * ld];
             x[row + (int64_t)c * ld] = gs_row(b[row + (int64_t)c * ld], acc[c], dg, omega, xi);
         }
     }
@@ -1454,6 +1503,42 @@
     block_sums_store<kNormWaves, D>(sums, red, wave, lane, bb, partials);
 }
 
+template <int D, int C16>
+__global__ __launch_bounds__(kNormWaves * 64, 8) void residual_norm_slices_head(const int64_t* __restrict__ slice_ptr, const int* __restrict__ col,
+                                                               const double* __restrict__ val, const double* __restrict__ diag,
+                                                               const double* __restrict__ b, const double* __restrict__ x,
+                                                               const double* __restrict__ weight, int ld, int n_slices, double* __restrict__ partials,
+                                                               const unsigned* __restrict__ col16, const int* __restrict__ win_base, int c16_arg,
+                                                               double* __restrict__ xh, int hb, int he, double omega) {
+    __shared__ double red[kNormWaves][2 * D];
+    const int wave = threadIdx.x >> 6, lane = threadIdx.x & 63;
+    int nblk = gridDim.x, bb = blockIdx.x;
+    if ((nblk & 7) == 0) bb = (bb & 7) * (nblk >> 3) + (bb >> 3);
+    const int s = __builtin_amdgcn_readfirstlane(bb * kNormWaves + wave);
+    double sums[2 * D];
+#pragma unroll
+    for (int c = 0; c < 2 * D; ++c) sums[c] = 0.0;
+    if (s < n_slices) {
+        const int row = s * 64 + lane;
+        double acc[D];
+        row_dot_sel<double, D, C16>(slice_ptr, col, col16, win_base, c16_arg, val, x, ld, s, lane, acc);
+        const double dg = diag[row];
+        const double w = weight ? weight[row] : 1.0;
+        const bool head = s >= hb && s < he;
+        const int64_t hrows = (int64_t)(he - hb) * 64;
+#pragma unroll
+        for (int c = 0; c < D; ++c) {
+            const double bi = b[row + (int64_t)c * ld];
+            const double xi = x[row + (int64_t)c * ld];
+            const double r = row_ax(acc[c], dg, xi) - bi;
+            sums[2 * c] = norm_term(r, w);
+            sums[2 * c + 1] = norm_term(bi, w);
+            if (head) xh[(row - hb * 64) + c * hrows] = omega == 1.0 ? gs_row(bi, acc[c], dg) : gs_row(bi, acc[c], dg, omega, xi);
+        }
+    }
+    block_sums_store<kNormWaves, D>(sums, red, wave, lane, bb, partials);
+}
+
 __global__ void add_correction(const float* __restrict__ e, double* __restrict__ x, int64_t n) {
     const int64_t i = (int64_t)blockIdx.x * blockDim.x + threadIdx.x;
     if (i < n) x[i] += (double)e[i];
diff --git a/include/gravomg_hip.h b/include/gravomg_hip.h
--- a/include/gravomg_hip.h
+++ b/include/gravomg_hip.h
@@ -57,6 +57,7 @@
     int speculate_head;
     int uniform_slices;
     int color_ahead;
+    int fold_head;
     int accelerate;
 } gmg_config;
 
```
